# succinctlabs/sp1

Measured on NVIDIA H100. Metric: riscv_cycles_proven_per_second_core, higher is better.
Workload: dtype u32 KoalaBear (Montgomery) / ext4

## Files before the change

### sp1_b200/csrc/zerocheck.cu

```cuda
#include "ctx.cuh"
#include "challenger.cuh"
#include "hostfield.hpp"
#include "kb31.cuh"
#include <algorithm>
#include <memory>
#include <vector>

#include "machine.cuh"
#include "zc_lower.hpp"
#include "sumcheck.cuh"

namespace {

using kb::Ext;
using hf::E4;

constexpr int ZC_BLOCK = 128;
constexpr int ZC_LOCAL_REGS = 128;
constexpr int ZC_GLOBAL_REGS = 1024;
constexpr unsigned ZC_GLOBAL_MAXB = 132 * 2;
constexpr size_t ZC_MAX_PIECES = 16;

template <class K> struct Ops;
template <> struct Ops<uint32_t> {
    static __device__ __forceinline__ uint32_t zero() { return 0; }
    static __device__ __forceinline__ uint32_t from_base(uint32_t x) { return x; }
    static __device__ __forceinline__ uint32_t add(uint32_t a, uint32_t b) { return kb::add(a, b); }
    static __device__ __forceinline__ uint32_t sub(uint32_t a, uint32_t b) { return kb::sub(a, b); }
    static __device__ __forceinline__ uint32_t mul(uint32_t a, uint32_t b) { return kb::mul(a, b); }
    static __device__ __forceinline__ uint32_t load(const uint32_t* p, uint64_t i) { return __ldg(p + i); }
    static __device__ __forceinline__ Ext scale(const Ext& e, uint32_t k) { return kb::ext_mul_base(e, k); }
};
template <> struct Ops<Ext> {
    static __device__ __forceinline__ Ext zero() { return kb::ext_zero(); }
    static __device__ __forceinline__ Ext from_base(uint32_t x) { return kb::ext_from_base(x); }
    static __device__ __forceinline__ Ext add(const Ext& a, const Ext& b) { return kb::ext_add(a, b); }
    static __device__ __forceinline__ Ext sub(const Ext& a, const Ext& b) { return kb::ext_sub(a, b); }
    static __device__ __forceinline__ Ext mul(const Ext& a, const Ext& b) { return kb::ext_mul(a, b); }
    static __device__ __forceinline__ Ext load(const Ext* p, uint64_t i) { return kb::ext_load(reinterpret_cast<const uint32_t*>(p + i)); }
    static __device__ __forceinline__ Ext scale(const Ext& e, const Ext& k) { return kb::ext_mul(e, k); }
};

struct ZcJob {
    const void* main; const void* prep; const uint32_t* alpha_pows; uint64_t h;
    uint32_t blk_start, nblk, chip, columns;
    uint32_t zc_begin, zc_end;
    const void* batch;
};
static_assert(sizeof(ZcJob) == 64, "ZcJob layout");
struct ZcFixJob {
    const void* main; const void* prep; uint32_t* out; uint64_t h;
    uint32_t main_w, prep_w, blk_start, pad;
};

template <class J>
__device__ __forceinline__ int find_job(const J* __restrict__ jobs, int n, uint32_t blk) {
    int lo = 0, hi = n - 1;
    while (lo < hi) {
        int mid = (lo + hi + 1) >> 1;
        if (jobs[mid].blk_start <= blk) lo = mid; else hi = mid - 1;
    }
    return lo;
}

enum { RF_SMEM = 0, RF_LOCAL = 1, RF_GLOBAL = 2 };
template <class K, int RF, int NODES = 3> struct RegFile;
template <class K, int NODES> struct RegFile<K, RF_SMEM, NODES> {
    K* base;
    __device__ __forceinline__ RegFile(unsigned char* smem, void*, uint32_t) : base(reinterpret_cast<K*>(smem) + threadIdx.x) {}
    __device__ __forceinline__ K get(uint32_t r, int n) const { return base[(r * NODES + n) * ZC_BLOCK]; }
    __device__ __forceinline__ void set(uint32_t r, int n, const K& v) { base[(r * NODES + n) * ZC_BLOCK] = v; }
};
template <class K, int NODES> struct RegFile<K, RF_LOCAL, NODES> {
    K regs[ZC_LOCAL_REGS * NODES];
    __device__ __forceinline__ RegFile(unsigned char*, void*, uint32_t) {}
    __device__ __forceinline__ K get(uint32_t r, int n) const { return regs[r * NODES + n]; }
    __device__ __forceinline__ void set(uint32_t r, int n, const K& v) { regs[r * NODES + n] = v; }
};
template <class K, int NODES> struct RegFile<K, RF_GLOBAL, NODES> {
    K* base;
    __device__ __forceinline__ RegFile(unsigned char*, void* ws, uint32_t ws_regs)
        : base(static_cast<K*>(ws) + (size_t)blockIdx.x * ws_regs * NODES * ZC_BLOCK + threadIdx.x) {}
    __device__ __forceinline__ K get(uint32_t r, int n) const { return base[(size_t)(r * NODES + n) * ZC_BLOCK]; }
    __device__ __forceinline__ void set(uint32_t r, int n, const K& v) { base[(size_t)(r * NODES + n) * ZC_BLOCK] = v; }
};

template <class K, int N0>
__device__ __forceinline__ void load_nodes(const K* __restrict__ base, uint32_t col, uint64_t h, uint64_t i, K (&v)[3]) {
    using O = Ops<K>;
    const K* c = base + (uint64_t)col * h;
    const K z = O::load(c, 2 * i);
    const K o = (2 * i + 1 < h) ? O::load(c, 2 * i + 1) : O::zero();
    const K d = O::sub(o, z);
    const K d2 = O::add(d, d);
    if (N0 == 0) v[0] = z;
    v[1] = O::add(z, d2);
    v[2] = O::add(v[1], d2);
}

template <class K, int RF, bool FIRST>
__global__ void __launch_bounds__(ZC_BLOCK) zc_sum_kernel(const ZcJob* __restrict__ jobs, int n_jobs, const ChipProg* __restrict__ chips,
                                                          const uint32_t* __restrict__ pv, const uint32_t* __restrict__ gkr_pows,
                                                          const uint32_t* __restrict__ E, uint32_t* __restrict__ partial,
                                                          void* __restrict__ ws, uint32_t ws_regs) {
    using O = Ops<K>;
    constexpr int N0 = FIRST ? 1 : 0;
    extern __shared__ __align__(16) unsigned char zc_smem[];
    __shared__ uint32_t red[5][4][ZC_BLOCK / 32];
    const ZcJob job = jobs[find_job(jobs, n_jobs, blockIdx.x)];
    const ChipProg& prog = chips[job.chip];
    const K* main = static_cast<const K*>(job.main);
    const K* prep = static_cast<const K*>(job.prep);
    const uint64_t h = job.h;
    const uint64_t terms = (h + 1) / 2;
    RegFile<K, RF> rf(zc_smem, ws, ws_regs);
    Ext acc[5];
#pragma unroll
    for (int a = 0; a < 5; a++) acc[a] = kb::ext_zero();
    const ZcInstr* __restrict__ zc = prog.zc + job.zc_begin;
    const uint32_t n_zc = job.zc_end - job.zc_begin;
    for (uint64_t i = (uint64_t)(blockIdx.x - job.blk_start) * ZC_BLOCK + threadIdx.x; i < terms; i += (uint64_t)job.nblk * ZC_BLOCK) {
        const Ext e = kb::ext_load(E + 4 * i);
        Ext row[3] = {kb::ext_zero(), kb::ext_zero(), kb::ext_zero()};
        ZcInstr in = n_zc ? zc[0] : ZcInstr{};
        for (uint32_t pc = 0; pc < n_zc; pc++) {
            const ZcInstr nxt = zc[pc + 1 < n_zc ? pc + 1 : pc];
            switch (in.op) {
                case ZC_LOAD_MAIN: case ZC_LOAD_PREP: {
                    K v[3];
                    load_nodes<K, N0>(in.op == ZC_LOAD_MAIN ? main : prep, (uint32_t)in.a | ((uint32_t)in.b << 16), h, i, v);
#pragma unroll
                    for (int n = N0; n < 3; n++) rf.set(in.out, n, v[n]);
                    break;
                }
                case ZC_CONST: { const K c = O::from_base(prog.consts[in.a]);
#pragma unroll
                    for (int n = N0; n < 3; n++) rf.set(in.out, n, c);
                    break; }
                case ZC_PUBLIC: { const K c = O::from_base(pv[prog.publics[in.a]]);
#pragma unroll
                    for (int n = N0; n < 3; n++) rf.set(in.out, n, c);
                    break; }
                case ZC_ADD: {
                    K r[3];
#pragma unroll
                    for (int n = N0; n < 3; n++) r[n] = O::add(rf.get(in.a, n), rf.get(in.b, n));
#pragma unroll
                    for (int n = N0; n < 3; n++) rf.set(in.out, n, r[n]);
                    break; }
                case ZC_SUB: {
                    K r[3];
#pragma unroll
                    for (int n = N0; n < 3; n++) r[n] = O::sub(rf.get(in.a, n), rf.get(in.b, n));
#pragma unroll
                    for (int n = N0; n < 3; n++) rf.set(in.out, n, r[n]);
                    break; }
                case ZC_MUL: {
                    K r[3];
#pragma unroll
                    for (int n = N0; n < 3; n++) r[n] = O::mul(rf.get(in.a, n), rf.get(in.b, n));
#pragma unroll
                    for (int n = N0; n < 3; n++) rf.set(in.out, n, r[n]);
                    break; }
                case ZC_NEG: {
                    K r[3];
#pragma unroll
                    for (int n = N0; n < 3; n++) r[n] = O::sub(O::zero(), rf.get(in.a, n));
#pragma unroll
                    for (int n = N0; n < 3; n++) rf.set(in.out, n, r[n]);
                    break; }
                case ZC_ASSERT: {
                    const Ext al = kb::ext_load(job.alpha_pows + 4 * in.b);
#pragma unroll
                    for (int n = N0; n < 3; n++) row[n] = kb::ext_add(row[n], O::scale(al, rf.get(in.a, n)));
                    break; }
                default: __trap();
            }
            in = nxt;
        }
#pragma unroll
        for (int n = N0; n < 3; n++) acc[n] = kb::ext_add(acc[n], kb::ext_mul(row[n], e));
        if (!job.columns) continue;
        Ext s0 = kb::ext_zero(), s1 = kb::ext_zero();
        const bool has_o = 2 * i + 1 < h;
        if (job.batch) {
            const uint32_t* B = static_cast<const uint32_t*>(job.batch);
            acc[3] = kb::ext_add(acc[3], kb::ext_mul(kb::ext_load(B + 8 * i), e));
            if (has_o) acc[4] = kb::ext_add(acc[4], kb::ext_mul(kb::ext_load(B + 8 * i + 4), e));
            continue;
        }
        for (uint32_t j = 0; j < prog.main_w; j++) {
            const Ext g = kb::ext_load(gkr_pows + 4 * j);
            const K* c = main + (uint64_t)j * h;
            s0 = kb::ext_add(s0, O::scale(g, O::load(c, 2 * i)));
            if (has_o) s1 = kb::ext_add(s1, O::scale(g, O::load(c, 2 * i + 1)));
        }
        for (uint32_t j = 0; j < prog.prep_w; j++) {
            const Ext g = kb::ext_load(gkr_pows + 4 * (prog.main_w + j));
            const K* c = prep + (uint64_t)j * h;
            s0 = kb::ext_add(s0, O::scale(g, O::load(c, 2 * i)));
            if (has_o) s1 = kb::ext_add(s1, O::scale(g, O::load(c, 2 * i + 1)));
        }
        acc[3] = kb::ext_add(acc[3], kb::ext_mul(s0, e));
        acc[4] = kb::ext_add(acc[4], kb::ext_mul(s1, e));
    }
    const int lane = threadIdx.x & 31, warp = threadIdx.x >> 5;
#pragma unroll
    for (int a = 0; a < 5; a++)
#pragma unroll
        for (int l = 0; l < 4; l++) {
            uint32_t v = acc[a].c[l];
            for (int s = 16; s > 0; s >>= 1) v = kb::add(v, __shfl_down_sync(0xffffffffu, v, s));
            if (lane == 0) red[a][l][warp] = v;
        }
    __syncthreads();
    if (threadIdx.x < 36) {
        const int node = threadIdx.x / 12, slot = (threadIdx.x >> 2) % 3, l = threadIdx.x & 3;
        const int a = slot == 0 ? node : (node == 0 ? 2 + slot : -1);
        uint32_t v = 0;
        if (a >= 0)
            for (int w = 0; w < ZC_BLOCK / 32; w++) v = kb::add(v, red[a][l][w]);
        partial[(uint64_t)blockIdx.x * 36 + threadIdx.x] = v;
    }
}

__global__ void __launch_bounds__(128) zc_reduce_kernel(const ZcJob* __restrict__ jobs, const uint32_t* __restrict__ partial, uint32_t* __restrict__ out,
                                                        Mail mail) {
    const ZcJob job = jobs[blockIdx.x];
    __shared__ uint32_t red[36][4];
    const int slot = threadIdx.x >> 2, part = threadIdx.x & 3;
    for (int w = slot; w < 36; w += 32) {
        uint32_t v = 0;
        for (uint32_t b = part; b < job.nblk; b += 4) v = kb::add(v, partial[(uint64_t)(job.blk_start + b) * 36 + w]);
        red[w][part] = v;
    }
    __syncthreads();
    if (threadIdx.x < 36) {
        const uint32_t* r = red[threadIdx.x];
        out[blockIdx.x * 36 + threadIdx.x] = kb::add(kb::add(r[0], r[1]), kb::add(r[2], r[3]));
    }
    sp1_mail_done(mail);
}

template <class K>
__global__ void __launch_bounds__(256) zc_fix_kernel(const ZcFixJob* __restrict__ jobs, int n_jobs, Ext alpha) {
    using O = Ops<K>;
    const ZcFixJob job = jobs[find_job(jobs, n_jobs, blockIdx.x)];
    const uint64_t h = job.h, nh = (h + 1) / 2;
    const uint32_t bpc = (uint32_t)((nh + 255) / 256);
    const uint32_t lb = blockIdx.x - job.blk_start;
    const uint64_t j = lb / bpc;
    const uint64_t i = (uint64_t)(lb - (uint32_t)j * bpc) * 256 + threadIdx.x;
    if (i >= nh) return;
    const uint64_t t = j * nh + i;
    const K* in = j < job.main_w ? static_cast<const K*>(job.main) + j * h : static_cast<const K*>(job.prep) + (j - job.main_w) * h;
    K a = O::load(in, 2 * i);
    K b = (2 * i + 1 < h) ? O::load(in, 2 * i + 1) : O::zero();
    Ext r;
    if constexpr (sizeof(K) == 4) r = kb::ext_add(kb::ext_from_base(a), kb::ext_mul_base(alpha, kb::sub(b, a)));
    else r = kb::ext_add(a, kb::ext_mul(alpha, kb::ext_sub(b, a)));
    kb::ext_store(job.out + 4 * t, r);
}

__global__ void __launch_bounds__(256) zc_batch0_kernel(const ZcFixJob* __restrict__ jobs, int n_jobs, const uint32_t* __restrict__ gkr_pows, Ext alpha) {
    const ZcFixJob job = jobs[find_job(jobs, n_jobs, blockIdx.x)];
    const uint64_t h = job.h, nh = (h + 1) / 2;
    const uint64_t i = (uint64_t)(blockIdx.x - job.blk_start) * 256 + threadIdx.x;
    if (i >= nh) return;
    const bool has_o = 2 * i + 1 < h;
    Ext sa = kb::ext_zero(), sd = kb::ext_zero();
    const uint32_t* main = static_cast<const uint32_t*>(job.main);
    const uint32_t* prep = static_cast<const uint32_t*>(job.prep);
    for (uint32_t j = 0; j < job.main_w + job.prep_w; j++) {
        const uint32_t* c = j < job.main_w ? main + (uint64_t)j * h : prep + (uint64_t)(j - job.main_w) * h;
        const uint32_t a = __ldg(c + 2 * i), b = has_o ? __ldg(c + 2 * i + 1) : 0u;
        const Ext g = kb::ext_load(gkr_pows + 4 * j);
        sa = kb::ext_add(sa, kb::ext_mul_base(g, a));
        sd = kb::ext_add(sd, kb::ext_mul_base(g, kb::sub(b, a)));
    }
    kb::ext_store(job.out + 4 * i, kb::ext_add(sa, kb::ext_mul(alpha, sd)));
}

struct ZcDbgJob {
    const uint32_t* main; const uint32_t* prep; uint64_t h;
    const uint32_t* rows;
    uint32_t* out;
    uint32_t* count;
    uint32_t n, blk_start, nblk, chip, cwords, pad;
};
static_assert(sizeof(ZcDbgJob) == 72, "ZcDbgJob layout");

template <int RF, bool LISTED>
__global__ void __launch_bounds__(ZC_BLOCK) zc_debug_kernel(const ZcDbgJob* __restrict__ jobs, int n_jobs, const ChipProg* __restrict__ chips,
                                                            const uint32_t* __restrict__ pv, void* __restrict__ ws, uint32_t ws_regs) {
    extern __shared__ __align__(16) unsigned char zc_smem[];
    const ZcDbgJob job = jobs[find_job(jobs, n_jobs, blockIdx.x)];
    const ChipProg& prog = chips[job.chip];
    RegFile<uint32_t, RF, 1> rf(zc_smem, ws, ws_regs);
    const ZcInstr* __restrict__ zc = prog.zc;
    const uint32_t n_zc = prog.n_zc, lane = threadIdx.x & 31;
    for (uint64_t t0 = (uint64_t)(blockIdx.x - job.blk_start) * ZC_BLOCK + (threadIdx.x - lane); t0 < job.n; t0 += (uint64_t)job.nblk * ZC_BLOCK) {
        const uint64_t t = t0 + lane;
        bool fail = false;
        if (t < job.n) {
            const uint64_t row = LISTED ? job.rows[t] : t;
            for (uint32_t pc = 0; pc < n_zc; pc++) {
                const ZcInstr in = zc[pc];
                switch (in.op) {
                    case ZC_LOAD_MAIN: rf.set(in.out, 0, __ldg(job.main + (uint64_t)((uint32_t)in.a | ((uint32_t)in.b << 16)) * job.h + row)); break;
                    case ZC_LOAD_PREP: rf.set(in.out, 0, __ldg(job.prep + (uint64_t)((uint32_t)in.a | ((uint32_t)in.b << 16)) * job.h + row)); break;
                    case ZC_CONST: rf.set(in.out, 0, prog.consts[in.a]); break;
                    case ZC_PUBLIC: rf.set(in.out, 0, pv[prog.publics[in.a]]); break;
                    case ZC_ADD: rf.set(in.out, 0, kb::add(rf.get(in.a, 0), rf.get(in.b, 0))); break;
                    case ZC_SUB: rf.set(in.out, 0, kb::sub(rf.get(in.a, 0), rf.get(in.b, 0))); break;
                    case ZC_MUL: rf.set(in.out, 0, kb::mul(rf.get(in.a, 0), rf.get(in.b, 0))); break;
                    case ZC_NEG: rf.set(in.out, 0, kb::neg(rf.get(in.a, 0))); break;
                    case ZC_ASSERT:
                        if (rf.get(in.a, 0)) {
                            fail = true;
                            if (LISTED) job.out[t * job.cwords + (in.b >> 5)] |= 1u << (in.b & 31);
                        }
                        break;
                    default: __trap();
                }
            }
        }
        if (!LISTED) {
            const uint32_t bits = __ballot_sync(0xffffffffu, fail);
            if (lane == 0 && bits) { job.out[t0 >> 5] = bits; atomicAdd(job.count, (uint32_t)__popc(bits)); }
        }
    }
}

struct ZcDbgSelect { const uint32_t* bits; uint32_t* rows; uint32_t n_words, take; };
__global__ void __launch_bounds__(32) zc_debug_select_kernel(const ZcDbgSelect* __restrict__ jobs) {
    const ZcDbgSelect s = jobs[blockIdx.x];
    const uint32_t lane = threadIdx.x;
    uint32_t taken = 0;
    for (uint32_t w0 = 0; w0 < s.n_words && taken < s.take; w0 += 32) {
        uint32_t word = w0 + lane < s.n_words ? s.bits[w0 + lane] : 0u;
        const uint32_t c = __popc(word);
        uint32_t incl = c;
        for (int d = 1; d < 32; d <<= 1) {
            const uint32_t x = __shfl_up_sync(0xffffffffu, incl, d);
            if (lane >= (uint32_t)d) incl += x;
        }
        for (uint32_t rank = taken + incl - c; word && rank < s.take; rank++, word &= word - 1)
            s.rows[rank] = (w0 + lane) * 32 + (uint32_t)(__ffs(word) - 1);
        taken += __shfl_sync(0xffffffffu, incl, 31);
    }
}

E4 host_eval_zero_row(const HostProg& p, const uint32_t* pv, const std::vector<E4>& powers, uint32_t n_regs) {
    std::vector<uint32_t> regs(n_regs ? n_regs : 1, 0);
    for (const DagInstr& in : p.instrs) {
        switch (in.opcode) {
            case BC_LOAD_LEAF: regs[in.out] = 0; break;
            case BC_LOAD_CONST: regs[in.out] = p.consts[in.a]; break;
            case BC_LOAD_PUBLIC: regs[in.out] = pv[p.publics[in.a]]; break;
            case BC_ADD_F: regs[in.out] = hf::add(regs[in.a], regs[in.b]); break;
            case BC_SUB_F: regs[in.out] = hf::sub(regs[in.a], regs[in.b]); break;
            case BC_MUL_F: regs[in.out] = hf::mul(regs[in.a], regs[in.b]); break;
            case BC_NEG_F: regs[in.out] = hf::neg(regs[in.a]); break;
        }
    }
    E4 acc;
    for (size_t i = 0; i < p.assert_regs.size(); i++) acc = acc + powers[p.assert_alphas[i]] * regs[p.assert_regs[i]];
    return acc;
}

struct VGeq {
    uint32_t threshold = 0; E4 geq_c, eq_c;
    VGeq fix_last(const E4& a) const {
        VGeq r; r.threshold = threshold >> 1; r.geq_c = geq_c;
        r.eq_c = (threshold & 1) == 0 ? (E4::one() - a) * eq_c : a * (eq_c + geq_c) - geq_c;
        return r;
    }
    E4 at(uint64_t idx) const { return idx < threshold ? E4() : (idx == threshold ? eq_c + geq_c : geq_c); }
};

}

sp1b200_machine::~sp1b200_machine() {
    if (interactions) sp1b200_free_interactions(interactions);
    cudaFree(d_arena);
    cudaFree(d_zc_arena);
    cudaFree(d_chips);
}

extern "C" {

sp1b200_err sp1b200_machine_create(sp1b200_ctx* ctx, const uint32_t* h_blob, uint64_t n_words, sp1b200_machine** out) { SP1_DEVICE_GUARD(ctx);
    auto m = std::make_unique<sp1b200_machine>();
    SP1_CUDA(cudaMalloc((void**)&m->d_arena, n_words * 4 + 16));
    SP1_CUDA(cudaMemcpyAsync(m->d_arena, h_blob, n_words * 4, cudaMemcpyHostToDevice, ctx->stream));
    const uint32_t* b = h_blob;
    const uint32_t* end = h_blob + n_words;
    auto dev = [&](const uint32_t* hp) { return m->d_arena + (hp - h_blob); };
    if (n_words < 1 || !h_blob) return sp1b200_set_error("machine_create: empty blob");
    uint32_t n = *b++;
    for (uint32_t c = 0; c < n; c++) {
        if ((uint64_t)(end - b) < 9) return sp1b200_set_error("machine_create: truncated blob (header of chip %u)", c);
        ChipProg p{}; HostProg hp;
        p.main_w = *b++; p.prep_w = *b++; p.n_constraints = *b++; p.n_regs = *b++;
        const uint64_t ni = *b++, nl = *b++, nc = *b++, np = *b++, na = *b++;
        if (2 * ni + 2 * nl + nc + np + 2 * na > (uint64_t)(end - b)) return sp1b200_set_error("machine_create: truncated blob (chip %u)", c);
        if (p.n_regs > 65536) return sp1b200_set_error("machine_create: chip %u declares %u registers (16-bit register indices)", c, p.n_regs);
        p.n_instrs = (uint32_t)ni; p.n_asserts = (uint32_t)na;
        p.instrs = reinterpret_cast<const DagInstr*>(dev(b)); hp.instrs.resize(ni); memcpy(hp.instrs.data(), b, ni * 8); b += 2 * ni;
        p.leaves = reinterpret_cast<const LeafRef*>(dev(b)); hp.leaves.resize(nl); memcpy(hp.leaves.data(), b, nl * 8); b += 2 * nl;
        p.consts = dev(b); hp.consts.assign(b, b + nc); b += nc;
        p.publics = dev(b); hp.publics.assign(b, b + np); b += np;
        p.assert_regs = dev(b); hp.assert_regs.assign(b, b + na); b += na;
        p.assert_alphas = dev(b); hp.assert_alphas.assign(b, b + na); b += na;
        for (const LeafRef& l : hp.leaves) {
            if (l.source != LEAF_MAIN && l.source != LEAF_PREP) return sp1b200_set_error("machine_create: chip %u: leaf source %u (expected 2 = preprocessed or 4 = main)", c, l.source);
            if (l.col >= (l.source == LEAF_MAIN ? p.main_w : p.prep_w)) return sp1b200_set_error("machine_create: chip %u: leaf column %u outside the %s width", c, l.col, l.source == LEAF_MAIN ? "main" : "preprocessed");
        }
        for (size_t k = 0; k < hp.instrs.size(); k++) {
            const DagInstr& in = hp.instrs[k];
            if (in.out >= p.n_regs) return sp1b200_set_error("machine_create: chip %u instr %zu: output register %u >= n_regs %u", c, k, in.out, p.n_regs);
            bool ok = true;
            switch (in.opcode) {
                case BC_LOAD_LEAF: ok = in.a < nl; break;
                case BC_LOAD_CONST: ok = in.a < nc; break;
                case BC_LOAD_PUBLIC: ok = in.a < np; break;
                case BC_ADD_F: case BC_SUB_F: case BC_MUL_F: ok = in.a < p.n_regs && in.b < p.n_regs; break;
                case BC_NEG_F: ok = in.a < p.n_regs; break;
                default: return sp1b200_set_error("machine_create: chip %u instr %zu: unknown opcode %u", c, k, in.opcode);
            }
            if (!ok) return sp1b200_set_error("machine_create: chip %u instr %zu: operand out of range (opcode %u, a %u, b %u)", c, k, in.opcode, in.a, in.b);
        }
        for (size_t k = 0; k < hp.assert_regs.size(); k++) {
            if (hp.assert_regs[k] >= p.n_regs) return sp1b200_set_error("machine_create: chip %u assert %zu: register %u >= n_regs %u", c, k, hp.assert_regs[k], p.n_regs);
            if (hp.assert_alphas[k] >= p.n_constraints) return sp1b200_set_error("machine_create: chip %u assert %zu: alpha index %u >= n_constraints %u", c, k, hp.assert_alphas[k], p.n_constraints);
        }
        m->chips.push_back(p); m->host.push_back(std::move(hp));
    }
    {
        std::vector<uint32_t> widths;
        for (auto& c : m->chips) { widths.push_back(c.main_w); widths.push_back(c.prep_w); }
        widths.push_back(0);
        m->interactions = sp1b200_parse_interactions(b, end, n, widths.data());
        if (!m->interactions) return sp1b200_last_error();
    }
    std::vector<ZcInstr> all;
    std::vector<size_t> zc_off(n);
    for (uint32_t c = 0; c < n; c++) {
        ZcLowered L = zc_lower(m->host[c]);
        if (!L.error.empty()) return sp1b200_set_error("machine_create: chip %u: %s", c, L.error.c_str());
        zc_off[c] = all.size();
        m->chips[c].n_zc = (uint32_t)L.instrs.size();
        m->chips[c].zc_regs = L.n_regs;
        all.insert(all.end(), L.instrs.begin(), L.instrs.end());
        const size_t na = m->host[c].assert_regs.size();
        const size_t np_ = std::min<size_t>(ZC_MAX_PIECES, na / 4);
        if (np_ >= 2 && L.instrs.size() >= 128) {
            for (size_t q = 0; q < np_; q++) {
                ZcLowered P = zc_lower(m->host[c], 24, na * q / np_, na * (q + 1) / np_);
                if (!P.error.empty()) return sp1b200_set_error("machine_create: chip %u: %s", c, P.error.c_str());
                m->host[c].zc_pieces.emplace_back((uint32_t)(all.size() - zc_off[c]), (uint32_t)P.instrs.size());
                m->chips[c].zc_regs = std::max(m->chips[c].zc_regs, P.n_regs);
                all.insert(all.end(), P.instrs.begin(), P.instrs.end());
            }
        }
    }
    SP1_CUDA(cudaMalloc(&m->d_zc_arena, all.size() * sizeof(ZcInstr) + 16));
    if (!all.empty()) SP1_CUDA(cudaMemcpyAsync(m->d_zc_arena, all.data(), all.size() * sizeof(ZcInstr), cudaMemcpyHostToDevice, ctx->stream));
    for (uint32_t c = 0; c < n; c++) m->chips[c].zc = static_cast<const ZcInstr*>(m->d_zc_arena) + zc_off[c];
    SP1_CUDA(cudaMalloc((void**)&m->d_chips, (n ? n : 1) * sizeof(ChipProg)));
    if (n) SP1_CUDA(cudaMemcpyAsync(m->d_chips, m->chips.data(), n * sizeof(ChipProg), cudaMemcpyHostToDevice, ctx->stream));
    SP1_CUDA(cudaStreamSynchronize(ctx->stream));
    *out = m.release();
    return nullptr;
}
void sp1b200_machine_free(sp1b200_ctx*, sp1b200_machine* m) { delete m; }
uint32_t sp1b200_machine_chip_regs(const sp1b200_machine* m, uint32_t chip) { return chip < m->chips.size() ? m->chips[chip].zc_regs : 0; }
uint32_t sp1b200_machine_num_chips(const sp1b200_machine* m) { return (uint32_t)m->chips.size(); }

sp1b200_err sp1b200_zerocheck(sp1b200_ctx* ctx, const sp1b200_machine* m, const uint64_t* h_heights, const uint32_t* const* d_main,
                              const uint32_t* const* d_prep, const uint32_t* h_pv, uint32_t n_pv, const uint32_t* h_gkr_point,
                              const uint32_t* h_alpha, const uint32_t* h_gamma, const uint32_t* h_claims, uint32_t* h_chal, uint32_t* h_out,
                              uint64_t cap, uint64_t* h_words) { SP1_DEVICE_GUARD(ctx);
    const uint32_t mlr = ctx->params.max_log_row_count;
    const size_t nchips = m->chips.size();
    for (size_t k = 0; k < nchips; k++)
        for (uint32_t pi : m->host[k].publics)
            if (pi >= n_pv) return sp1b200_set_error("zerocheck: chip %zu reads public value %u but only %u were passed", k, pi, n_pv);
    cudaStream_t st = ctx->stream;
    DevFree mem(ctx);
    HostChallenger ch;
    SP1_TRY(ch.init(ctx, h_chal));
    PhaseTimer t_all(ctx, "zerocheck.total");
    HostAccum acc_wait(ctx, "zerocheck.host_wait"), acc_math(ctx, "zerocheck.host_math"), acc_setup(ctx, "zerocheck.host_setup");
    auto t_setup = std::make_unique<HostSpan>(acc_setup);
    const E4 alpha = E4::load(h_alpha), gamma = E4::load(h_gamma);

    struct St {
        uint64_t h;
        std::vector<E4> zeta; E4 eq_adj = E4::one(), pra; VGeq vg;
    };
    std::vector<St> S(nchips);
    size_t maxc = 0, maxw = 0, total_w = 0, total_c = 0;
    for (auto& c : m->chips) {
        maxc = std::max<size_t>(maxc, c.n_constraints); maxw = std::max<size_t>(maxw, c.main_w + c.prep_w);
        total_w += c.main_w + c.prep_w; total_c += c.n_constraints ? c.n_constraints : 1;
    }
    std::vector<E4> pw(maxc ? maxc : 1); pw[0] = E4::one();
    for (size_t i = 1; i < pw.size(); i++) pw[i] = pw[i - 1] * alpha;
    std::vector<E4> gw(maxw ? maxw : 1); gw[0] = gamma;
    for (size_t i = 1; i < gw.size(); i++) gw[i] = gw[i - 1] * gamma;
    uint32_t *d_pv, *d_gw, *d_ap;
    SP1_TRY(mem.alloc((void**)&d_pv, (n_pv ? n_pv : 1) * 4));
    if (n_pv) SP1_CUDA(cudaMemcpyAsync(d_pv, h_pv, n_pv * 4, cudaMemcpyHostToDevice, st));
    SP1_TRY(mem.alloc((void**)&d_gw, gw.size() * 16));
    SP1_CUDA(cudaMemcpyAsync(d_gw, gw.data(), gw.size() * 16, cudaMemcpyHostToDevice, st));
    std::vector<E4> gp(mlr);
    for (uint32_t i = 0; i < mlr; i++) gp[i] = E4::load(h_gkr_point + 4 * i);
    std::vector<E4> all_ap; all_ap.reserve(total_c);
    std::vector<size_t> ap_off(nchips), woff(nchips);
    std::vector<uint64_t> boff0(nchips), boff1(nchips);
    uint64_t b0 = 0, b1 = 0; size_t wsum = 0;
    for (size_t k = 0; k < nchips; k++) {
        const ChipProg& p = m->chips[k];
        St& s = S[k];
        s.h = h_heights[k];
        if (s.h > ((uint64_t)1 << mlr)) return sp1b200_set_error("zerocheck: chip %zu height exceeds 2^%u", k, mlr);
        if (p.zc_regs > ZC_GLOBAL_REGS) return sp1b200_set_error("zerocheck: chip %zu needs %u live registers (> %d)", k, p.zc_regs, ZC_GLOBAL_REGS);
        s.zeta = gp;
        std::vector<E4> rev(pw.begin(), pw.begin() + p.n_constraints);
        std::reverse(rev.begin(), rev.end());
        ap_off[k] = all_ap.size();
        all_ap.insert(all_ap.end(), rev.begin(), rev.end());
        if (rev.empty()) all_ap.push_back(E4());
        s.pra = host_eval_zero_row(m->host[k], h_pv, rev, p.n_regs);
        s.vg.threshold = (uint32_t)s.h; s.vg.geq_c = E4::one();
        const uint64_t nh = (s.h + 1) / 2;
        const size_t w = p.main_w + p.prep_w;
        boff0[k] = b0; b0 += (uint64_t)(w + 1) * nh * 4;
        boff1[k] = b1; b1 += (uint64_t)(w + 1) * ((nh + 1) / 2) * 4;
        woff[k] = wsum; wsum += w;
    }
    SP1_TRY(mem.alloc((void**)&d_ap, all_ap.size() * 16));
    SP1_CUDA(cudaMemcpyAsync(d_ap, all_ap.data(), all_ap.size() * 16, cudaMemcpyHostToDevice, st));
    uint32_t *d_buf[2], *d_final;
    SP1_TRY(mem.alloc((void**)&d_buf[0], b0 * 4 + 16));
    SP1_TRY(mem.alloc((void**)&d_buf[1], b1 * 4 + 16));
    SP1_TRY(mem.alloc((void**)&d_final, (wsum ? wsum : 1) * 16));
    uint32_t *d_point, *d_E[2];
    SP1_TRY(mem.alloc((void**)&d_point, mlr * 16));
    SP1_CUDA(cudaMemcpyAsync(d_point, h_gkr_point, mlr * 16, cudaMemcpyHostToDevice, st));
    SP1_TRY(mem.alloc((void**)&d_E[0], ((size_t)16 << (mlr - 1))));
    SP1_TRY(mem.alloc((void**)&d_E[1], ((size_t)16 << (mlr > 1 ? mlr - 2 : 0))));
    SP1_TRY(launch_eq_table(ctx, d_point, (int)mlr - 1, d_E[0]));
    int ecur = 0;

    static const uint32_t TIER_REGS[3] = {8, 16, 32};
    auto tier_of = [&](uint32_t regs) { for (int t = 0; t < 3; t++) if (regs <= TIER_REGS[t]) return t; return regs <= (uint32_t)ZC_LOCAL_REGS ? 3 : 4; };
    size_t ws_bytes = 0;
    struct Launch { size_t job0; uint32_t n_jobs, blocks, regs; int tier; };
    struct RoundPlan { std::vector<Launch> sums; size_t fix0; uint32_t fix_jobs, fix_blocks; std::vector<uint32_t> chip_of_job; size_t job0; };
    std::vector<RoundPlan> plan(mlr);
    std::vector<ZcJob> jobs;
    std::vector<ZcFixJob> fjobs, bjobs;
    uint32_t batch_blocks = 0;
    const unsigned MAXB = 132 * 4;
    uint32_t max_blocks = 1, max_jobs = 1;
    {
        std::vector<uint64_t> hcur(nchips);
        for (size_t k = 0; k < nchips; k++) hcur[k] = S[k].h;
        for (uint32_t rd = 0; rd < mlr; rd++) {
            RoundPlan& R = plan[rd];
            R.job0 = jobs.size();
            auto in_main = [&](size_t k) -> const void* {
                if (rd == 0) return d_main[k];
                return (rd & 1 ? d_buf[0] + boff0[k] : d_buf[1] + boff1[k]);
            };
            auto in_prep = [&](size_t k) -> const void* {
                const ChipProg& p = m->chips[k];
                if (rd == 0) return p.prep_w ? d_prep[k] : nullptr;
                return static_cast<const uint32_t*>(in_main(k)) + (uint64_t)p.main_w * hcur[k] * 4;
            };
            auto in_batch = [&](size_t k) -> const void* {
                if (rd == 0) return nullptr;
                const ChipProg& p = m->chips[k];
                return static_cast<const uint32_t*>(in_main(k)) + (uint64_t)(p.main_w + p.prep_w) * hcur[k] * 4;
            };
            uint32_t blocks_round = 0;
            for (int tier = 0; tier < 5; tier++) {
                Launch Lc{jobs.size(), 0, 0, 0, tier};
                for (size_t k = 0; k < nchips; k++) {
                    const ChipProg& p = m->chips[k];
                    if (!hcur[k] || tier_of(p.zc_regs) != tier) continue;
                    unsigned nb = blocks_for((hcur[k] + 1) / 2, ZC_BLOCK);
                    if (nb > MAXB) nb = MAXB;
                    if (tier == 4 && nb > ZC_GLOBAL_MAXB) nb = ZC_GLOBAL_MAXB;
                    const auto& pieces = m->host[k].zc_pieces;
                    if (nb <= 16 && !pieces.empty()) {
                        for (size_t q = 0; q < pieces.size(); q++) {
                            ZcJob j{in_main(k), in_prep(k), d_ap + 4 * ap_off[k], hcur[k], Lc.blocks, nb, (uint32_t)k, q == 0 ? 1u : 0u,
                                    pieces[q].first, pieces[q].first + pieces[q].second, in_batch(k)};
                            jobs.push_back(j);
                            R.chip_of_job.push_back((uint32_t)k);
                            Lc.n_jobs++; Lc.blocks += nb;
                        }
                    } else {
                        ZcJob j{in_main(k), in_prep(k), d_ap + 4 * ap_off[k], hcur[k], Lc.blocks, nb, (uint32_t)k, 1u, 0u, p.n_zc, in_batch(k)};
                        jobs.push_back(j);
                        R.chip_of_job.push_back((uint32_t)k);
                        Lc.n_jobs++; Lc.blocks += nb;
                    }
                    Lc.regs = std::max(Lc.regs, p.zc_regs);
                }
                if (Lc.n_jobs) {
                    R.sums.push_back(Lc); blocks_round += Lc.blocks;
                    if (tier == 4) ws_bytes = std::max(ws_bytes, (size_t)Lc.blocks * Lc.regs * 3 * ZC_BLOCK * 16);
                }
            }
            max_blocks = std::max(max_blocks, blocks_round);
            max_jobs = std::max<uint32_t>(max_jobs, (uint32_t)R.chip_of_job.size());
            R.fix0 = fjobs.size(); R.fix_jobs = 0; R.fix_blocks = 0;
            for (size_t k = 0; k < nchips; k++) {
                const ChipProg& p = m->chips[k];
                if (!hcur[k]) continue;
                const uint64_t nh = (hcur[k] + 1) / 2;
                uint32_t* out = rd + 1 == mlr ? d_final + 4 * woff[k] : (rd & 1 ? d_buf[1] + boff1[k] : d_buf[0] + boff0[k]);
                const uint32_t fold_b = (rd > 0 && rd + 1 < mlr) ? 1u : 0u;
                ZcFixJob f{in_main(k), in_prep(k), out, hcur[k], p.main_w, p.prep_w + fold_b, R.fix_blocks, 0};
                fjobs.push_back(f);
                R.fix_jobs++; R.fix_blocks += blocks_for(nh, 256) * (p.main_w + p.prep_w + fold_b);
                if (rd == 0 && mlr > 1) {
                    ZcFixJob bj{d_main[k], m->chips[k].prep_w ? d_prep[k] : nullptr, d_buf[0] + boff0[k] + (uint64_t)(p.main_w + p.prep_w) * nh * 4, hcur[k],
                                p.main_w, p.prep_w, batch_blocks, 0};
                    bjobs.push_back(bj);
                    batch_blocks += blocks_for(nh, 256);
                }
                hcur[k] = nh;
            }
        }
    }
    ZcJob* d_jobs; ZcFixJob *d_fjobs, *d_bjobs; uint32_t *d_partial, *d_sums;
    SP1_TRY(mem.alloc((void**)&d_jobs, (jobs.size() + 1) * sizeof(ZcJob)));
    SP1_TRY(mem.alloc((void**)&d_fjobs, (fjobs.size() + 1) * sizeof(ZcFixJob)));
    SP1_TRY(mem.alloc((void**)&d_bjobs, (bjobs.size() + 1) * sizeof(ZcFixJob)));
    if (!bjobs.empty()) SP1_CUDA(cudaMemcpyAsync(d_bjobs, bjobs.data(), bjobs.size() * sizeof(ZcFixJob), cudaMemcpyHostToDevice, st));
    if (!jobs.empty()) SP1_CUDA(cudaMemcpyAsync(d_jobs, jobs.data(), jobs.size() * sizeof(ZcJob), cudaMemcpyHostToDevice, st));
    if (!fjobs.empty()) SP1_CUDA(cudaMemcpyAsync(d_fjobs, fjobs.data(), fjobs.size() * sizeof(ZcFixJob), cudaMemcpyHostToDevice, st));
    SP1_TRY(mem.alloc((void**)&d_partial, (size_t)max_blocks * 36 * 4));
    if ((size_t)max_jobs * 36 > SP1_MAIL_WORDS) return sp1b200_set_error("zerocheck: %u chips exceed the mailbox payload", max_jobs);
    d_sums = sp1b200_mail_dev(ctx);
    SP1_CUDA(cudaMemsetAsync(d_final, 0, (wsum ? wsum : 1) * 16, st));
    void* d_ws = nullptr;
    if (ws_bytes) SP1_TRY(mem.alloc(&d_ws, ws_bytes));
    auto launch_sum = [&](const Launch& Lc, bool ext, uint32_t* part) -> sp1b200_err {
        auto go = [&](auto kern, size_t smem) -> sp1b200_err {
            if (smem > 32 * 1024) SP1_CUDA(cudaFuncSetAttribute(kern, cudaFuncAttributeMaxDynamicSharedMemorySize, (int)smem));
            SP1_LAUNCH(ctx, kern, Lc.blocks, ZC_BLOCK, smem, d_jobs + Lc.job0, (int)Lc.n_jobs, m->d_chips, d_pv, d_gw, d_E[ecur], part, d_ws,
                       Lc.regs);
            return nullptr;
        };
        if (Lc.tier == 4) return ext ? go(zc_sum_kernel<Ext, RF_GLOBAL, false>, 0) : go(zc_sum_kernel<uint32_t, RF_GLOBAL, true>, 0);
        if (Lc.tier == 3) return ext ? go(zc_sum_kernel<Ext, RF_LOCAL, false>, 0) : go(zc_sum_kernel<uint32_t, RF_LOCAL, true>, 0);
        const size_t regs = Lc.regs;
        return ext ? go(zc_sum_kernel<Ext, RF_SMEM, false>, regs * 3 * ZC_BLOCK * 16) : go(zc_sum_kernel<uint32_t, RF_SMEM, true>, regs * 3 * ZC_BLOCK * 4);
    };

    t_setup.reset();
    E4 lambda; ch.sample_ext(lambda.c);
    std::vector<E4> round_claims(nchips);
    E4 claimed_sum;
    for (size_t k = 0; k < nchips; k++) { round_claims[k] = E4::load(h_claims + 4 * k); claimed_sum = claimed_sum * lambda + round_claims[k]; }
    std::vector<uint32_t> words;
    words.push_back(mlr);
    std::vector<E4> point;
    std::vector<E4> ys((size_t)nchips * 4);
    std::vector<uint32_t> hs((size_t)max_jobs * 36);
    std::vector<E4> chip_sums(nchips * 9);
    const E4 two = E4::from_base(hf::to_monty(2)), four = E4::from_base(hf::to_monty(4)), three = E4::from_base(hf::to_monty(3));
    for (uint32_t rd = 0; rd < mlr; rd++) {
        const RoundPlan& R = plan[rd];
        {
            uint32_t blk = 0, seq = 0; size_t jb = 0;
            for (const Launch& Lc : R.sums) {
                SP1_TRY(launch_sum(Lc, rd > 0, d_partial + (size_t)blk * 36));
                const Mail mail = sp1b200_mail_next(ctx); seq = mail.seq;
                SP1_LAUNCH(ctx, zc_reduce_kernel, Lc.n_jobs, 128, 0, d_jobs + Lc.job0, d_partial + (size_t)blk * 36, d_sums + jb * 36, mail);
                blk += Lc.blocks; jb += Lc.n_jobs;
            }
            if (jb) {
                HostSpan sp(acc_wait);
                SP1_TRY(sp1b200_mail_wait(ctx, seq));
                memcpy(hs.data(), sp1b200_mail_host(ctx), jb * 36 * 4);
            }
        }
        HostSpan sp_math(acc_math);
        std::fill(chip_sums.begin(), chip_sums.end(), E4());
        for (size_t j = 0; j < R.chip_of_job.size(); j++)
            for (int w9 = 0; w9 < 9; w9++) chip_sums[(size_t)R.chip_of_job[j] * 9 + w9] = chip_sums[(size_t)R.chip_of_job[j] * 9 + w9] + E4::load(&hs[j * 36 + 4 * w9]);
        const E4 last = gp[mlr - 1 - rd];
        const E4 bnode = (E4::one() - last) * hf::inv(E4::one() - (last + last));
        const E4 nodes[5] = {E4(), E4::one(), two, four, bnode};
        E4 basis[5][5];
        hf::lagrange_basis<5>(nodes, basis);
        const E4 f0 = E4::one() - last, f2 = last * hf::to_monty(3) - E4::one(), f4 = last * hf::to_monty(7) - three;
        E4 Y[4];
        for (size_t k = 0; k < nchips; k++) {
            St& s = S[k];
            E4* y = &ys[4 * k];
            if (s.h == 0) { y[0] = y[1] = y[2] = y[3] = E4(); }
            else {
                const E4* q = &chip_sums[k * 9];
                const E4 A = q[1], B = q[2];
                E4 y0 = q[0] + A;
                E4 y2 = q[3] + (B + B) - A;
                E4 y4 = q[6] + B * four - A * three;
                const uint64_t th = (s.h + 1) / 2 - 1;
                const uint64_t esize = (uint64_t)1 << (s.zeta.size() - 1);
                E4 eth;
                if (th < esize) {
                    const size_t kk = s.zeta.size() - 1;
                    eth = E4::one();
                    for (size_t t = 0; t < kk; t++) eth = eth * (((th >> (kk - 1 - t)) & 1) ? s.zeta[t] : E4::one() - s.zeta[t]);
                }
                const E4 msb = s.eq_adj * eth;
                const E4 v0 = s.vg.fix_last(E4()).at(th), v2 = s.vg.fix_last(two).at(th), v4 = s.vg.fix_last(four).at(th);
                y0 = y0 * (f0 * s.eq_adj) - s.pra * v0 * msb * f0;
                y2 = y2 * (f2 * s.eq_adj) - s.pra * v2 * msb * f2;
                y4 = y4 * (f4 * s.eq_adj) - s.pra * v4 * msb * f4;
                y[0] = y0; y[1] = round_claims[k] - y0; y[2] = y2; y[3] = y4;
            }
            for (int i = 0; i < 4; i++) Y[i] = (k ? Y[i] * lambda : E4()) + y[i];
        }
        E4 rlc[5];
        for (int c5 = 0; c5 < 5; c5++) for (int i = 0; i < 4; i++) rlc[c5] = rlc[c5] + basis[i][c5] * Y[i];
        for (auto& c : rlc) ch.observe_n(c.c, 4);
        words.push_back(5);
        for (auto& c : rlc) words.insert(words.end(), c.c, c.c + 4);
        E4 a; ch.sample_ext(a.c);
        point.insert(point.begin(), a);
        const Ext da = to_ext(a);
        if (R.fix_jobs) {
            if (rd == 0) {
                SP1_LAUNCH(ctx, zc_fix_kernel<uint32_t>, R.fix_blocks, 256, 0, d_fjobs + R.fix0, (int)R.fix_jobs, da);
                if (!bjobs.empty()) SP1_LAUNCH(ctx, zc_batch0_kernel, batch_blocks, 256, 0, d_bjobs, (int)bjobs.size(), d_gw, da);
            } else SP1_LAUNCH(ctx, zc_fix_kernel<Ext>, R.fix_blocks, 256, 0, d_fjobs + R.fix0, (int)R.fix_jobs, da);
        }
        E4 La[4];
        for (int i = 0; i < 4; i++) La[i] = hf::eval_poly<5>(basis[i], a);
        for (size_t k = 0; k < nchips; k++) {
            St& s = S[k];
            const E4* y = &ys[4 * k];
            round_claims[k] = y[0] * La[0] + y[1] * La[1] + y[2] * La[2] + y[3] * La[3];
            s.vg = s.vg.fix_last(a);
            if (s.h == 0) continue;
            s.eq_adj = s.eq_adj * (a * last + (E4::one() - a) * (E4::one() - last));
            s.zeta.pop_back();
            s.h = (s.h + 1) / 2;
        }
        if (rd + 1 < mlr) {
            const uint64_t n_out = (uint64_t)1 << (mlr - 2 - rd);
            SP1_TRY(launch_halve_eq(ctx, d_E[ecur], n_out, d_E[ecur ^ 1]));
            ecur ^= 1;
        }
    }
    E4 final_eval;
    for (auto& c : round_claims) final_eval = final_eval * lambda + c;
    words.insert(words.end(), claimed_sum.c, claimed_sum.c + 4);
    for (auto& x : point) words.insert(words.end(), x.c, x.c + 4);
    words.insert(words.end(), final_eval.c, final_eval.c + 4);
    std::vector<uint32_t> fin((wsum ? wsum : 1) * 4);
    SP1_CUDA(cudaMemcpyAsync(fin.data(), d_final, fin.size() * 4, cudaMemcpyDeviceToHost, st));
    SP1_CUDA(cudaStreamSynchronize(st));
    ch.observe(hf::to_monty(nchips));
    for (size_t k = 0; k < nchips; k++) {
        const ChipProg& p = m->chips[k];
        const uint32_t* mv = &fin[4 * woff[k]];
        const uint32_t* pvv = mv + 4 * (size_t)p.main_w;
        ch.observe(hf::to_monty(p.prep_w)); ch.observe_n(pvv, (size_t)p.prep_w * 4);
        ch.observe(hf::to_monty(p.main_w)); ch.observe_n(mv, (size_t)p.main_w * 4);
        words.insert(words.end(), pvv, pvv + (size_t)p.prep_w * 4);
        words.insert(words.end(), mv, mv + (size_t)p.main_w * 4);
    }
    t_all.stop();
    ch.store(h_chal);
    if (h_words) *h_words = words.size();
    if (words.size() > cap) return sp1b200_set_error("zerocheck: output needs %zu words, capacity %llu", words.size(), (unsigned long long)cap);
    if (h_out) memcpy(h_out, words.data(), words.size() * 4);
    return nullptr;
}

}

sp1b200_err sp1b200_debug_constraints_device(sp1b200_ctx* ctx, const sp1b200_machine* m, const uint64_t* h_heights, const uint32_t* const* d_main,
                                             const uint32_t* const* d_prep, const uint32_t* h_pv, uint32_t n_pv, uint32_t max_rows,
                                             std::vector<uint32_t>& words) {
    const size_t nchips = m->chips.size();
    for (size_t k = 0; k < nchips; k++) {
        for (uint32_t pi : m->host[k].publics)
            if (pi >= n_pv) return sp1b200_set_error("debug_constraints: chip %zu reads public value %u but only %u were passed", k, pi, n_pv);
        if (m->chips[k].zc_regs > ZC_GLOBAL_REGS)
            return sp1b200_set_error("debug_constraints: chip %zu needs %u live registers (> %d)", k, m->chips[k].zc_regs, ZC_GLOBAL_REGS);
    }
    cudaStream_t st = ctx->stream;
    DevFree mem(ctx);
    PhaseTimer t_all(ctx, "debug_constraints.total");
    uint32_t* d_pv;
    SP1_TRY(mem.alloc((void**)&d_pv, (n_pv ? n_pv : 1) * 4));
    if (n_pv) SP1_CUDA(cudaMemcpyAsync(d_pv, h_pv, n_pv * 4, cudaMemcpyHostToDevice, st));
    static const uint32_t TIER_REGS[3] = {8, 16, 32};
    auto tier_of = [&](uint32_t regs) { for (int t = 0; t < 3; t++) if (regs <= TIER_REGS[t]) return t; return regs <= (uint32_t)ZC_LOCAL_REGS ? 3 : 4; };
    struct Launch { size_t job0; uint32_t n_jobs, blocks, regs; int tier; };
    auto plan = [&](std::vector<ZcDbgJob>& jobs, std::vector<Launch>& launches, size_t& ws_bytes, auto n_of, auto fill) {
        for (int tier = 0; tier < 5; tier++) {
            Launch Lc{jobs.size(), 0, 0, 0, tier};
            for (size_t k = 0; k < nchips; k++) {
                const uint64_t n = n_of(k);
                if (!n || tier_of(m->chips[k].zc_regs) != tier) continue;
                unsigned nb = std::min<unsigned>(blocks_for(n, ZC_BLOCK), 132 * 4);
                if (tier == 4) nb = std::min(nb, ZC_GLOBAL_MAXB);
                ZcDbgJob j{};
                j.main = d_main[k]; j.prep = m->chips[k].prep_w ? d_prep[k] : nullptr; j.h = h_heights[k];
                j.n = (uint32_t)n; j.blk_start = Lc.blocks; j.nblk = nb; j.chip = (uint32_t)k;
                fill(k, j);
                jobs.push_back(j);
                Lc.n_jobs++; Lc.blocks += nb; Lc.regs = std::max(Lc.regs, m->chips[k].zc_regs);
            }
            if (Lc.n_jobs) {
                launches.push_back(Lc);
                if (tier == 4) ws_bytes = std::max(ws_bytes, (size_t)Lc.blocks * Lc.regs * ZC_BLOCK * 4);
            }
        }
    };
    auto run = [&](const std::vector<ZcDbgJob>& jobs, const std::vector<Launch>& launches, size_t ws_bytes, bool listed) -> sp1b200_err {
        ZcDbgJob* d_jobs;
        void* d_ws = nullptr;
        SP1_TRY(mem.alloc((void**)&d_jobs, (jobs.size() + 1) * sizeof(ZcDbgJob)));
        if (!jobs.empty()) SP1_CUDA(cudaMemcpyAsync(d_jobs, jobs.data(), jobs.size() * sizeof(ZcDbgJob), cudaMemcpyHostToDevice, st));
        if (ws_bytes) SP1_TRY(mem.alloc(&d_ws, ws_bytes));
        for (const Launch& Lc : launches) {
            auto go = [&](auto kern, size_t smem) -> sp1b200_err {
                SP1_LAUNCH(ctx, kern, Lc.blocks, ZC_BLOCK, smem, d_jobs + Lc.job0, (int)Lc.n_jobs, m->d_chips, d_pv, d_ws, Lc.regs);
                return nullptr;
            };
            sp1b200_err e;
            if (Lc.tier == 4) e = listed ? go(zc_debug_kernel<RF_GLOBAL, true>, 0) : go(zc_debug_kernel<RF_GLOBAL, false>, 0);
            else if (Lc.tier == 3) e = listed ? go(zc_debug_kernel<RF_LOCAL, true>, 0) : go(zc_debug_kernel<RF_LOCAL, false>, 0);
            else e = listed ? go(zc_debug_kernel<RF_SMEM, true>, (size_t)Lc.regs * ZC_BLOCK * 4)
                            : go(zc_debug_kernel<RF_SMEM, false>, (size_t)Lc.regs * ZC_BLOCK * 4);
            SP1_TRY(e);
        }
        return nullptr;
    };

    std::vector<uint64_t> bm_off(nchips);
    uint64_t bm_words = 0;
    for (size_t k = 0; k < nchips; k++) { bm_off[k] = bm_words; bm_words += (h_heights[k] + 31) / 32; }
    uint32_t *d_bm, *d_cnt;
    SP1_TRY(mem.alloc((void**)&d_bm, (bm_words ? bm_words : 1) * 4));
    SP1_TRY(mem.alloc((void**)&d_cnt, (nchips ? nchips : 1) * 4));
    SP1_CUDA(cudaMemsetAsync(d_bm, 0, (bm_words ? bm_words : 1) * 4, st));
    SP1_CUDA(cudaMemsetAsync(d_cnt, 0, (nchips ? nchips : 1) * 4, st));
    {
        std::vector<ZcDbgJob> jobs; std::vector<Launch> launches; size_t ws = 0;
        plan(jobs, launches, ws, [&](size_t k) { return h_heights[k]; },
             [&](size_t k, ZcDbgJob& j) { j.out = d_bm + bm_off[k]; j.count = d_cnt + k; });
        SP1_TRY(run(jobs, launches, ws, false));
    }
    std::vector<uint32_t> cnt(nchips);
    if (nchips) SP1_CUDA(cudaMemcpyAsync(cnt.data(), d_cnt, nchips * 4, cudaMemcpyDeviceToHost, st));
    SP1_CUDA(cudaStreamSynchronize(st));

    std::vector<uint64_t> row_off(nchips), cbm_off(nchips);
    std::vector<uint32_t> take(nchips), cwords(nchips);
    uint64_t n_rows = 0, n_cbm = 0;
    std::vector<ZcDbgSelect> sel;
    uint32_t* d_rows;
    for (size_t k = 0; k < nchips; k++) {
        take[k] = std::min(cnt[k], max_rows);
        cwords[k] = (m->chips[k].n_constraints + 31) / 32;
        row_off[k] = n_rows; n_rows += take[k];
        cbm_off[k] = n_cbm; n_cbm += (uint64_t)take[k] * cwords[k];
    }
    SP1_TRY(mem.alloc((void**)&d_rows, (n_rows ? n_rows : 1) * 4));
    std::vector<uint32_t> rows(n_rows), cbm(n_cbm);
    if (n_rows) {
        for (size_t k = 0; k < nchips; k++)
            if (take[k]) sel.push_back(ZcDbgSelect{d_bm + bm_off[k], d_rows + row_off[k], (uint32_t)((h_heights[k] + 31) / 32), take[k]});
        ZcDbgSelect* d_sel;
        uint32_t* d_cbm;
        SP1_TRY(mem.alloc((void**)&d_sel, sel.size() * sizeof(ZcDbgSelect)));
        SP1_TRY(mem.alloc((void**)&d_cbm, (n_cbm ? n_cbm : 1) * 4));
        SP1_CUDA(cudaMemcpyAsync(d_sel, sel.data(), sel.size() * sizeof(ZcDbgSelect), cudaMemcpyHostToDevice, st));
        SP1_CUDA(cudaMemsetAsync(d_cbm, 0, (n_cbm ? n_cbm : 1) * 4, st));
        SP1_LAUNCH(ctx, zc_debug_select_kernel, (unsigned)sel.size(), 32, 0, d_sel);
        std::vector<ZcDbgJob> jobs; std::vector<Launch> launches; size_t ws = 0;
        plan(jobs, launches, ws, [&](size_t k) { return (uint64_t)take[k]; },
             [&](size_t k, ZcDbgJob& j) { j.rows = d_rows + row_off[k]; j.out = d_cbm + cbm_off[k]; j.cwords = cwords[k]; });
        SP1_TRY(run(jobs, launches, ws, true));
        SP1_CUDA(cudaMemcpyAsync(rows.data(), d_rows, n_rows * 4, cudaMemcpyDeviceToHost, st));
        if (n_cbm) SP1_CUDA(cudaMemcpyAsync(cbm.data(), d_cbm, n_cbm * 4, cudaMemcpyDeviceToHost, st));
        SP1_CUDA(cudaStreamSynchronize(st));
    }
    t_all.stop();
    words.assign(1, 0);
    for (size_t k = 0; k < nchips; k++) {
        if (!cnt[k]) continue;
        words[0]++;
        words.push_back((uint32_t)k); words.push_back(cnt[k]); words.push_back(take[k]);
        for (uint32_t i = 0; i < take[k]; i++) {
            words.push_back(rows[row_off[k] + i]);
            const size_t n_at = words.size();
            words.push_back(0);
            const uint32_t* b = &cbm[cbm_off[k] + (uint64_t)i * cwords[k]];
            for (uint32_t c = 0; c < m->chips[k].n_constraints; c++)
                if ((b[c >> 5] >> (c & 31)) & 1) { words.push_back(c); words[n_at]++; }
        }
    }
    return nullptr;
}
```

Measured before the change: 64.76 million.

## Evaluate first two zerocheck rounds on a 2D grid in one base-field pass

Adds a grid kernel that reads four rows at once and evaluates constraints on a 2D node grid, so round 0 and round 1 sums both come from a single base-field pass over the trace. The host derives both rounds' univariate evaluations from 16 accumulated sums. A fold2 kernel then folds two variables at once, replacing the separate round-0 fix, the batch0 kernel, the round-1 extension-field sum pass and one eq-halving. The cost is six nodes per interpreter pass, done twice, which means more register or shared-memory pressure and more interpreted work in the first round.

```diff
diff --git a/sp1_b200/csrc/zc_grid.hpp b/sp1_b200/csrc/zc_grid.hpp
--- /dev/null
+++ b/sp1_b200/csrc/zc_grid.hpp
@@ -0,0 +1,29 @@
+#pragma once
+#include "hostfield.hpp"
+#include <cstdint>
+
+inline void zc_grid_round0(const hf::E4* g, const hf::E4& z, uint64_t h, const hf::E4& pad, hf::E4* out) {
+    using hf::E4;
+    const E4 z0 = E4::one() - z;
+    const E4 skip = (h % 4 == 1 || h % 4 == 2) ? z * pad : E4();
+    for (int i = 0; i < 9; i++) out[i] = E4();
+    out[3] = z0 * g[0] + z * g[1] - skip;
+    out[6] = z0 * g[4] + z * g[5] - skip;
+    out[1] = z0 * g[12] + z * g[14];
+    out[2] = z0 * g[13] + z * g[15];
+}
+
+inline void zc_grid_round1(const hf::E4* g, const hf::E4& a0, uint64_t h, const hf::E4& pad, hf::E4* out) {
+    using hf::E4;
+    const E4 nodes[4] = {E4(), E4::one(), E4::from_base(hf::to_monty(2)), E4::from_base(hf::to_monty(4))};
+    E4 basis[4][4];
+    hf::lagrange_basis<4>(nodes, basis);
+    E4 L[4];
+    for (int i = 0; i < 4; i++) L[i] = hf::eval_poly<4>(basis[i], a0);
+    for (int i = 0; i < 9; i++) out[i] = E4();
+    out[0] = L[2] * g[0] + L[3] * g[4] + (h % 4 == 1 ? L[1] * pad : E4());
+    out[3] = L[0] * g[8] + L[1] * g[10] + L[2] * g[2] + L[3] * g[6];
+    out[6] = L[0] * g[9] + L[1] * g[11] + L[2] * g[3] + L[3] * g[7];
+    out[1] = g[12] + a0 * (g[13] - g[12]);
+    out[2] = g[14] + a0 * (g[15] - g[14]);
+}
diff --git a/sp1_b200/csrc/zerocheck.cu b/sp1_b200/csrc/zerocheck.cu
--- a/sp1_b200/csrc/zerocheck.cu
+++ b/sp1_b200/csrc/zerocheck.cu
@@ -8,6 +8,7 @@
 
 #include "machine.cuh"
 #include "zc_lower.hpp"
+#include "zc_grid.hpp"
 #include "sumcheck.cuh"
 
 namespace {
@@ -51,6 +52,7 @@
 struct ZcFixJob {
     const void* main; const void* prep; uint32_t* out; uint64_t h;
     uint32_t main_w, prep_w, blk_start, pad;
+    const uint32_t* corners;
 };
 
 template <class J>
@@ -98,6 +100,70 @@
     v[2] = O::add(v[1], d2);
 }
 
+template <class K, int RF, int NODES, int N0, class Load>
+__device__ __forceinline__ void zc_interpret(const ZcJob& job, const ChipProg& prog, const uint32_t* __restrict__ pv,
+                                             RegFile<K, RF, NODES>& rf, const Load& load, Ext (&row)[NODES]) {
+    using O = Ops<K>;
+    const ZcInstr* __restrict__ zc = prog.zc + job.zc_begin;
+    const uint32_t n_zc = job.zc_end - job.zc_begin;
+    ZcInstr in = n_zc ? zc[0] : ZcInstr{};
+    for (uint32_t pc = 0; pc < n_zc; pc++) {
+        const ZcInstr nxt = zc[pc + 1 < n_zc ? pc + 1 : pc];
+        switch (in.op) {
+            case ZC_LOAD_MAIN: case ZC_LOAD_PREP: {
+                K v[NODES];
+                load(in.op == ZC_LOAD_MAIN, (uint32_t)in.a | ((uint32_t)in.b << 16), v);
+#pragma unroll
+                for (int n = N0; n < NODES; n++) rf.set(in.out, n, v[n]);
+                break;
+            }
+            case ZC_CONST: { const K c = O::from_base(prog.consts[in.a]);
+#pragma unroll
+                for (int n = N0; n < NODES; n++) rf.set(in.out, n, c);
+                break; }
+            case ZC_PUBLIC: { const K c = O::from_base(pv[prog.publics[in.a]]);
+#pragma unroll
+                for (int n = N0; n < NODES; n++) rf.set(in.out, n, c);
+                break; }
+            case ZC_ADD: {
+                K r[NODES];
+#pragma unroll
+                for (int n = N0; n < NODES; n++) r[n] = O::add(rf.get(in.a, n), rf.get(in.b, n));
+#pragma unroll
+                for (int n = N0; n < NODES; n++) rf.set(in.out, n, r[n]);
+                break; }
+            case ZC_SUB: {
+                K r[NODES];
+#pragma unroll
+                for (int n = N0; n < NODES; n++) r[n] = O::sub(rf.get(in.a, n), rf.get(in.b, n));
+#pragma unroll
+                for (int n = N0; n < NODES; n++) rf.set(in.out, n, r[n]);
+                break; }
+            case ZC_MUL: {
+                K r[NODES];
+#pragma unroll
+                for (int n = N0; n < NODES; n++) r[n] = O::mul(rf.get(in.a, n), rf.get(in.b, n));
+#pragma unroll
+                for (int n = N0; n < NODES; n++) rf.set(in.out, n, r[n]);
+                break; }
+            case ZC_NEG: {
+                K r[NODES];
+#pragma unroll
+                for (int n = N0; n < NODES; n++) r[n] = O::sub(O::zero(), rf.get(in.a, n));
+#pragma unroll
+                for (int n = N0; n < NODES; n++) rf.set(in.out, n, r[n]);
+                break; }
+            case ZC_ASSERT: {
+                const Ext al = kb::ext_load(job.alpha_pows + 4 * in.b);
+#pragma unroll
+                for (int n = N0; n < NODES; n++) row[n] = kb::ext_add(row[n], O::scale(al, rf.get(in.a, n)));
+                break; }
+            default: __trap();
+        }
+        in = nxt;
+    }
+}
+
 template <class K, int RF, bool FIRST>
 __global__ void __launch_bounds__(ZC_BLOCK) zc_sum_kernel(const ZcJob* __restrict__ jobs, int n_jobs, const ChipProg* __restrict__ chips,
                                                           const uint32_t* __restrict__ pv, const uint32_t* __restrict__ gkr_pows,
@@ -117,67 +183,11 @@
     Ext acc[5];
 #pragma unroll
     for (int a = 0; a < 5; a++) acc[a] = kb::ext_zero();
-    const ZcInstr* __restrict__ zc = prog.zc + job.zc_begin;
-    const uint32_t n_zc = job.zc_end - job.zc_begin;
     for (uint64_t i = (uint64_t)(blockIdx.x - job.blk_start) * ZC_BLOCK + threadIdx.x; i < terms; i += (uint64_t)job.nblk * ZC_BLOCK) {
         const Ext e = kb::ext_load(E + 4 * i);
         Ext row[3] = {kb::ext_zero(), kb::ext_zero(), kb::ext_zero()};
-        ZcInstr in = n_zc ? zc[0] : ZcInstr{};
-        for (uint32_t pc = 0; pc < n_zc; pc++) {
-            const ZcInstr nxt = zc[pc + 1 < n_zc ? pc + 1 : pc];
-            switch (in.op) {
-                case ZC_LOAD_MAIN: case ZC_LOAD_PREP: {
-                    K v[3];
-                    load_nodes<K, N0>(in.op == ZC_LOAD_MAIN ? main : prep, (uint32_t)in.a | ((uint32_t)in.b << 16), h, i, v);
-#pragma unroll
-                    for (int n = N0; n < 3; n++) rf.set(in.out, n, v[n]);
-                    break;
-                }
-                case ZC_CONST: { const K c = O::from_base(prog.consts[in.a]);
-#pragma unroll
-                    for (int n = N0; n < 3; n++) rf.set(in.out, n, c);
-                    break; }
-                case ZC_PUBLIC: { const K c = O::from_base(pv[prog.publics[in.a]]);
-#pragma unroll
-                    for (int n = N0; n < 3; n++) rf.set(in.out, n, c);
-                    break; }
-                case ZC_ADD: {
-                    K r[3];
-#pragma unroll
-                    for (int n = N0; n < 3; n++) r[n] = O::add(rf.get(in.a, n), rf.get(in.b, n));
-#pragma unroll
-                    for (int n = N0; n < 3; n++) rf.set(in.out, n, r[n]);
-                    break; }
-                case ZC_SUB: {
-                    K r[3];
-#pragma unroll
-                    for (int n = N0; n < 3; n++) r[n] = O::sub(rf.get(in.a, n), rf.get(in.b, n));
-#pragma unroll
-                    for (int n = N0; n < 3; n++) rf.set(in.out, n, r[n]);
-                    break; }
-                case ZC_MUL: {
-                    K r[3];
-#pragma unroll
-                    for (int n = N0; n < 3; n++) r[n] = O::mul(rf.get(in.a, n), rf.get(in.b, n));
-#pragma unroll
-                    for (int n = N0; n < 3; n++) rf.set(in.out, n, r[n]);
-                    break; }
-                case ZC_NEG: {
-                    K r[3];
-#pragma unroll
-                    for (int n = N0; n < 3; n++) r[n] = O::sub(O::zero(), rf.get(in.a, n));
-#pragma unroll
-                    for (int n = N0; n < 3; n++) rf.set(in.out, n, r[n]);
-                    break; }
-                case ZC_ASSERT: {
-                    const Ext al = kb::ext_load(job.alpha_pows + 4 * in.b);
-#pragma unroll
-                    for (int n = N0; n < 3; n++) row[n] = kb::ext_add(row[n], O::scale(al, rf.get(in.a, n)));
-                    break; }
-                default: __trap();
-            }
-            in = nxt;
-        }
+        zc_interpret<K, RF, 3, N0>(job, prog, pv, rf, [&](bool is_main, uint32_t col, K (&v)[3]) { load_nodes<K, N0>(is_main ? main : prep, col, h, i, v); },
+                                   row);
 #pragma unroll
         for (int n = N0; n < 3; n++) acc[n] = kb::ext_add(acc[n], kb::ext_mul(row[n], e));
         if (!job.columns) continue;
@@ -224,20 +234,122 @@
     }
 }
 
+constexpr int ZC_GRID_WORDS = 64;
+constexpr int ZC_GRID_NODES = 6;
+template <int RF>
+__global__ void __launch_bounds__(ZC_BLOCK, 3) zc_grid_kernel(const ZcJob* __restrict__ jobs, int n_jobs, const ChipProg* __restrict__ chips,
+                                                           const uint32_t* __restrict__ pv, const uint32_t* __restrict__ gkr_pows,
+                                                           const uint32_t* __restrict__ E, uint32_t* __restrict__ partial,
+                                                           void* __restrict__ ws, uint32_t ws_regs) {
+    extern __shared__ __align__(16) unsigned char zc_smem[];
+    const ZcJob job = jobs[find_job(jobs, n_jobs, blockIdx.x)];
+    const ChipProg& prog = chips[job.chip];
+    const uint32_t* main = static_cast<const uint32_t*>(job.main);
+    const uint32_t* prep = static_cast<const uint32_t*>(job.prep);
+    const uint64_t h = job.h;
+    const uint64_t terms = (h + 3) / 4;
+    RegFile<uint32_t, RF, ZC_GRID_NODES> rf(zc_smem, ws, ws_regs);
+    Ext acc[16];
+#pragma unroll
+    for (int a = 0; a < 16; a++) acc[a] = kb::ext_zero();
+    for (uint64_t q = (uint64_t)(blockIdx.x - job.blk_start) * ZC_BLOCK + threadIdx.x; q < terms; q += (uint64_t)job.nblk * ZC_BLOCK) {
+        const Ext e = kb::ext_load(E + 4 * q);
+        const uint64_t r0 = 4 * q;
+        auto quad = [&](const uint32_t* c, uint32_t (&v)[4]) {
+#pragma unroll
+            for (int t = 0; t < 4; t++) v[t] = r0 + t < h ? __ldg(c + r0 + t) : 0u;
+        };
+#pragma unroll
+        for (int pass = 0; pass < 2; pass++) {
+            Ext row[ZC_GRID_NODES];
+#pragma unroll
+            for (int n = 0; n < ZC_GRID_NODES; n++) row[n] = kb::ext_zero();
+            zc_interpret<uint32_t, RF, ZC_GRID_NODES, 0>(job, prog, pv, rf, [&](bool is_main, uint32_t col, uint32_t (&v)[ZC_GRID_NODES]) {
+                uint32_t c[4];
+                quad((is_main ? main : prep) + (uint64_t)col * h, c);
+                const uint32_t d0 = kb::sub(c[1], c[0]), d1 = kb::sub(c[3], c[2]);
+                const uint32_t x0 = kb::add(d0, d0), x1 = kb::add(d1, d1);
+                const uint32_t a = kb::add(c[0], pass ? kb::add(x0, x0) : x0), b = kb::add(c[2], pass ? kb::add(x1, x1) : x1);
+                const uint32_t d = kb::sub(b, a), d2 = kb::add(d, d);
+                v[0] = a; v[1] = b; v[2] = kb::add(a, d2); v[3] = kb::add(v[2], d2);
+                const uint32_t dy = kb::sub(c[2 + pass], c[pass]), y2 = kb::add(dy, dy);
+                v[4] = kb::add(c[pass], y2); v[5] = kb::add(v[4], y2);
+            }, row);
+#pragma unroll
+            for (int n = 0; n < 4; n++) acc[4 * pass + n] = kb::ext_add(acc[4 * pass + n], kb::ext_mul(row[n], e));
+#pragma unroll
+            for (int n = 0; n < 2; n++) acc[8 + 2 * pass + n] = kb::ext_add(acc[8 + 2 * pass + n], kb::ext_mul(row[4 + n], e));
+        }
+        if (!job.columns) continue;
+        Ext s[4] = {kb::ext_zero(), kb::ext_zero(), kb::ext_zero(), kb::ext_zero()};
+        for (uint32_t j = 0; j < prog.main_w + prog.prep_w; j++) {
+            const Ext g = kb::ext_load(gkr_pows + 4 * j);
+            uint32_t c[4];
+            quad(j < prog.main_w ? main + (uint64_t)j * h : prep + (uint64_t)(j - prog.main_w) * h, c);
+#pragma unroll
+            for (int t = 0; t < 4; t++) s[t] = kb::ext_add(s[t], kb::ext_mul_base(g, c[t]));
+        }
+#pragma unroll
+        for (int t = 0; t < 4; t++) acc[12 + t] = kb::ext_add(acc[12 + t], kb::ext_mul(s[t], e));
+        if (job.batch) {
+            uint32_t* out = static_cast<uint32_t*>(const_cast<void*>(job.batch)) + 16 * q;
+#pragma unroll
+            for (int t = 0; t < 4; t++) kb::ext_store(out + 4 * t, s[t]);
+        }
+    }
+    block_reduce<16>(acc, partial, Mail{});
+}
+
+__global__ void __launch_bounds__(256) zc_fold2_kernel(const ZcFixJob* __restrict__ jobs, int n_jobs, Ext a0, Ext a1) {
+    const ZcFixJob job = jobs[find_job(jobs, n_jobs, blockIdx.x)];
+    const uint64_t h = job.h, nq = (h + 3) / 4;
+    const uint32_t bpc = (uint32_t)((nq + 255) / 256);
+    const uint32_t lb = blockIdx.x - job.blk_start;
+    const uint32_t j = lb / bpc;
+    const uint64_t q = (uint64_t)(lb - j * bpc) * 256 + threadIdx.x;
+    if (q >= nq) return;
+    const uint32_t w = job.main_w + job.prep_w;
+    const Ext a01 = kb::ext_mul(a0, a1);
+    auto col = [&](uint32_t k) {
+        return k < job.main_w ? static_cast<const uint32_t*>(job.main) + (uint64_t)k * h : static_cast<const uint32_t*>(job.prep) + (uint64_t)(k - job.main_w) * h;
+    };
+    auto coeffs = [&](uint32_t k, uint32_t (&d)[4]) {
+        const uint32_t* c = col(k);
+        uint32_t v[4];
+#pragma unroll
+        for (int t = 0; t < 4; t++) v[t] = 4 * q + t < h ? __ldg(c + 4 * q + t) : 0u;
+        d[0] = v[0]; d[1] = kb::sub(v[1], v[0]); d[2] = kb::sub(v[2], v[0]); d[3] = kb::sub(kb::sub(v[3], v[1]), d[2]);
+    };
+    Ext r;
+    if (j < w) {
+        uint32_t d[4];
+        coeffs(j, d);
+        r = kb::ext_add(kb::ext_add(kb::ext_from_base(d[0]), kb::ext_mul_base(a0, d[1])), kb::ext_add(kb::ext_mul_base(a1, d[2]), kb::ext_mul_base(a01, d[3])));
+    } else {
+        const uint32_t* c = job.corners + 16 * q;
+        const Ext s00 = kb::ext_load(c), s10 = kb::ext_load(c + 4), s01 = kb::ext_load(c + 8), s11 = kb::ext_load(c + 12);
+        const Ext d2 = kb::ext_sub(s01, s00);
+        const Ext d3 = kb::ext_sub(kb::ext_sub(s11, s10), d2);
+        r = kb::ext_add(kb::ext_add(s00, kb::ext_mul(a0, kb::ext_sub(s10, s00))), kb::ext_add(kb::ext_mul(a1, d2), kb::ext_mul(a01, d3)));
+    }
+    kb::ext_store(job.out + 4 * ((uint64_t)j * nq + q), r);
+}
+
+template <int WORDS>
 __global__ void __launch_bounds__(128) zc_reduce_kernel(const ZcJob* __restrict__ jobs, const uint32_t* __restrict__ partial, uint32_t* __restrict__ out,
                                                         Mail mail) {
     const ZcJob job = jobs[blockIdx.x];
-    __shared__ uint32_t red[36][4];
+    __shared__ uint32_t red[WORDS][4];
     const int slot = threadIdx.x >> 2, part = threadIdx.x & 3;
-    for (int w = slot; w < 36; w += 32) {
+    for (int w = slot; w < WORDS; w += 32) {
         uint32_t v = 0;
-        for (uint32_t b = part; b < job.nblk; b += 4) v = kb::add(v, partial[(uint64_t)(job.blk_start + b) * 36 + w]);
+        for (uint32_t b = part; b < job.nblk; b += 4) v = kb::add(v, partial[(uint64_t)(job.blk_start + b) * WORDS + w]);
         red[w][part] = v;
     }
     __syncthreads();
-    if (threadIdx.x < 36) {
+    if (threadIdx.x < WORDS) {
         const uint32_t* r = red[threadIdx.x];
-        out[blockIdx.x * 36 + threadIdx.x] = kb::add(kb::add(r[0], r[1]), kb::add(r[2], r[3]));
+        out[blockIdx.x * WORDS + threadIdx.x] = kb::add(kb::add(r[0], r[1]), kb::add(r[2], r[3]));
     }
     sp1_mail_done(mail);
 }
@@ -260,25 +372,6 @@
     if constexpr (sizeof(K) == 4) r = kb::ext_add(kb::ext_from_base(a), kb::ext_mul_base(alpha, kb::sub(b, a)));
     else r = kb::ext_add(a, kb::ext_mul(alpha, kb::ext_sub(b, a)));
     kb::ext_store(job.out + 4 * t, r);
-}
-
-__global__ void __launch_bounds__(256) zc_batch0_kernel(const ZcFixJob* __restrict__ jobs, int n_jobs, const uint32_t* __restrict__ gkr_pows, Ext alpha) {
-    const ZcFixJob job = jobs[find_job(jobs, n_jobs, blockIdx.x)];
-    const uint64_t h = job.h, nh = (h + 1) / 2;
-    const uint64_t i = (uint64_t)(blockIdx.x - job.blk_start) * 256 + threadIdx.x;
-    if (i >= nh) return;
-    const bool has_o = 2 * i + 1 < h;
-    Ext sa = kb::ext_zero(), sd = kb::ext_zero();
-    const uint32_t* main = static_cast<const uint32_t*>(job.main);
-    const uint32_t* prep = static_cast<const uint32_t*>(job.prep);
-    for (uint32_t j = 0; j < job.main_w + job.prep_w; j++) {
-        const uint32_t* c = j < job.main_w ? main + (uint64_t)j * h : prep + (uint64_t)(j - job.main_w) * h;
-        const uint32_t a = __ldg(c + 2 * i), b = has_o ? __ldg(c + 2 * i + 1) : 0u;
-        const Ext g = kb::ext_load(gkr_pows + 4 * j);
-        sa = kb::ext_add(sa, kb::ext_mul_base(g, a));
-        sd = kb::ext_add(sd, kb::ext_mul_base(g, kb::sub(b, a)));
-    }
-    kb::ext_store(job.out + 4 * i, kb::ext_add(sa, kb::ext_mul(alpha, sd)));
 }
 
 struct ZcDbgJob {
@@ -369,6 +462,13 @@
     return acc;
 }
 
+E4 eq_at(const std::vector<E4>& zeta, size_t kk, uint64_t idx) {
+    if (kk < 64 && idx >> kk) return E4();
+    E4 e = E4::one();
+    for (size_t t = 0; t < kk; t++) e = e * (((idx >> (kk - 1 - t)) & 1) ? zeta[t] : E4::one() - zeta[t]);
+    return e;
+}
+
 struct VGeq {
     uint32_t threshold = 0; E4 geq_c, eq_c;
     VGeq fix_last(const E4& a) const {
@@ -501,6 +601,7 @@
         std::vector<E4> zeta; E4 eq_adj = E4::one(), pra; VGeq vg;
     };
     std::vector<St> S(nchips);
+    const bool grid = mlr >= 2;
     size_t maxc = 0, maxw = 0, total_w = 0, total_c = 0;
     for (auto& c : m->chips) {
         maxc = std::max<size_t>(maxc, c.n_constraints); maxw = std::max<size_t>(maxw, c.main_w + c.prep_w);
@@ -519,8 +620,8 @@
     for (uint32_t i = 0; i < mlr; i++) gp[i] = E4::load(h_gkr_point + 4 * i);
     std::vector<E4> all_ap; all_ap.reserve(total_c);
     std::vector<size_t> ap_off(nchips), woff(nchips);
-    std::vector<uint64_t> boff0(nchips), boff1(nchips);
-    uint64_t b0 = 0, b1 = 0; size_t wsum = 0;
+    std::vector<uint64_t> boff0(nchips), boff1(nchips), coff(nchips);
+    uint64_t b0 = 0, b1 = 0, cw = 0; size_t wsum = 0;
     for (size_t k = 0; k < nchips; k++) {
         const ChipProg& p = m->chips[k];
         St& s = S[k];
@@ -535,10 +636,13 @@
         if (rev.empty()) all_ap.push_back(E4());
         s.pra = host_eval_zero_row(m->host[k], h_pv, rev, p.n_regs);
         s.vg.threshold = (uint32_t)s.h; s.vg.geq_c = E4::one();
-        const uint64_t nh = (s.h + 1) / 2;
+        const uint64_t nq = (s.h + 3) / 4;
         const size_t w = p.main_w + p.prep_w;
-        boff0[k] = b0; b0 += (uint64_t)(w + 1) * nh * 4;
-        boff1[k] = b1; b1 += (uint64_t)(w + 1) * ((nh + 1) / 2) * 4;
+        if (grid) {
+            boff0[k] = b0; b0 += (uint64_t)(w + 1) * ((nq + 1) / 2) * 4;
+            boff1[k] = b1; b1 += (uint64_t)(w + 1) * nq * 4;
+        }
+        coff[k] = cw; cw += nq * 16;
         woff[k] = wsum; wsum += w;
     }
     SP1_TRY(mem.alloc((void**)&d_ap, all_ap.size() * 16));
@@ -547,12 +651,16 @@
     SP1_TRY(mem.alloc((void**)&d_buf[0], b0 * 4 + 16));
     SP1_TRY(mem.alloc((void**)&d_buf[1], b1 * 4 + 16));
     SP1_TRY(mem.alloc((void**)&d_final, (wsum ? wsum : 1) * 16));
+    const bool keep_corners = grid && mlr > 2;
+    uint32_t* d_corners = nullptr;
+    if (keep_corners) SP1_TRY(mem.alloc((void**)&d_corners, cw * 4 + 16));
     uint32_t *d_point, *d_E[2];
+    const uint32_t e_bits = grid ? mlr - 2 : mlr - 1;
     SP1_TRY(mem.alloc((void**)&d_point, mlr * 16));
     SP1_CUDA(cudaMemcpyAsync(d_point, h_gkr_point, mlr * 16, cudaMemcpyHostToDevice, st));
-    SP1_TRY(mem.alloc((void**)&d_E[0], ((size_t)16 << (mlr - 1))));
-    SP1_TRY(mem.alloc((void**)&d_E[1], ((size_t)16 << (mlr > 1 ? mlr - 2 : 0))));
-    SP1_TRY(launch_eq_table(ctx, d_point, (int)mlr - 1, d_E[0]));
+    SP1_TRY(mem.alloc((void**)&d_E[0], ((size_t)16 << e_bits)));
+    SP1_TRY(mem.alloc((void**)&d_E[1], ((size_t)16 << (e_bits ? e_bits - 1 : 0))));
+    SP1_TRY(launch_eq_table(ctx, d_point, (int)e_bits, d_E[0]));
     int ecur = 0;
 
     static const uint32_t TIER_REGS[3] = {8, 16, 32};
@@ -562,8 +670,7 @@
     struct RoundPlan { std::vector<Launch> sums; size_t fix0; uint32_t fix_jobs, fix_blocks; std::vector<uint32_t> chip_of_job; size_t job0; };
     std::vector<RoundPlan> plan(mlr);
     std::vector<ZcJob> jobs;
-    std::vector<ZcFixJob> fjobs, bjobs;
-    uint32_t batch_blocks = 0;
+    std::vector<ZcFixJob> fjobs;
     const unsigned MAXB = 132 * 4;
     uint32_t max_blocks = 1, max_jobs = 1;
     {
@@ -582,21 +689,24 @@
                 return static_cast<const uint32_t*>(in_main(k)) + (uint64_t)p.main_w * hcur[k] * 4;
             };
             auto in_batch = [&](size_t k) -> const void* {
-                if (rd == 0) return nullptr;
+                if (rd == 0) return keep_corners ? d_corners + coff[k] : nullptr;
                 const ChipProg& p = m->chips[k];
                 return static_cast<const uint32_t*>(in_main(k)) + (uint64_t)(p.main_w + p.prep_w) * hcur[k] * 4;
             };
             uint32_t blocks_round = 0;
-            for (int tier = 0; tier < 5; tier++) {
+            const bool grid_pass = grid && rd == 0;
+            for (int tier = 0; tier < 5 && !(grid && rd == 1); tier++) {
                 Launch Lc{jobs.size(), 0, 0, 0, tier};
                 for (size_t k = 0; k < nchips; k++) {
                     const ChipProg& p = m->chips[k];
                     if (!hcur[k] || tier_of(p.zc_regs) != tier) continue;
-                    unsigned nb = blocks_for((hcur[k] + 1) / 2, ZC_BLOCK);
+                    unsigned nb = blocks_for(grid_pass ? (hcur[k] + 3) / 4 : (hcur[k] + 1) / 2, ZC_BLOCK);
                     if (nb > MAXB) nb = MAXB;
+                    if (grid_pass && nb > 132 * 3) nb = 132 * 3;
                     if (tier == 4 && nb > ZC_GLOBAL_MAXB) nb = ZC_GLOBAL_MAXB;
                     const auto& pieces = m->host[k].zc_pieces;
-                    if (nb <= 16 && !pieces.empty()) {
+                    const bool short_round = nb <= 16 || (!grid_pass && (hcur[k] + 1) / 2 <= 2ull * nb * ZC_BLOCK);
+                    if (short_round && !pieces.empty()) {
                         for (size_t q = 0; q < pieces.size(); q++) {
                             ZcJob j{in_main(k), in_prep(k), d_ap + 4 * ap_off[k], hcur[k], Lc.blocks, nb, (uint32_t)k, q == 0 ? 1u : 0u,
                                     pieces[q].first, pieces[q].first + pieces[q].second, in_batch(k)};
@@ -614,7 +724,7 @@
                 }
                 if (Lc.n_jobs) {
                     R.sums.push_back(Lc); blocks_round += Lc.blocks;
-                    if (tier == 4) ws_bytes = std::max(ws_bytes, (size_t)Lc.blocks * Lc.regs * 3 * ZC_BLOCK * 16);
+                    if (tier == 4) ws_bytes = std::max(ws_bytes, (size_t)Lc.blocks * Lc.regs * ZC_BLOCK * (grid_pass ? ZC_GRID_NODES * 4 : 3 * 16));
                 }
             }
             max_blocks = std::max(max_blocks, blocks_round);
@@ -625,40 +735,48 @@
                 if (!hcur[k]) continue;
                 const uint64_t nh = (hcur[k] + 1) / 2;
                 uint32_t* out = rd + 1 == mlr ? d_final + 4 * woff[k] : (rd & 1 ? d_buf[1] + boff1[k] : d_buf[0] + boff0[k]);
+                if (grid_pass) { hcur[k] = nh; continue; }
+                if (grid && rd == 1) {
+                    const uint32_t fold_b = rd + 1 < mlr ? 1u : 0u;
+                    ZcFixJob f{d_main[k], p.prep_w ? d_prep[k] : nullptr, out, S[k].h, p.main_w, p.prep_w, R.fix_blocks, fold_b,
+                               keep_corners ? d_corners + coff[k] : nullptr};
+                    fjobs.push_back(f);
+                    R.fix_jobs++; R.fix_blocks += blocks_for(nh, 256) * (p.main_w + p.prep_w + fold_b);
+                    hcur[k] = nh;
+                    continue;
+                }
                 const uint32_t fold_b = (rd > 0 && rd + 1 < mlr) ? 1u : 0u;
-                ZcFixJob f{in_main(k), in_prep(k), out, hcur[k], p.main_w, p.prep_w + fold_b, R.fix_blocks, 0};
+                ZcFixJob f{in_main(k), in_prep(k), out, hcur[k], p.main_w, p.prep_w + fold_b, R.fix_blocks, 0, nullptr};
                 fjobs.push_back(f);
                 R.fix_jobs++; R.fix_blocks += blocks_for(nh, 256) * (p.main_w + p.prep_w + fold_b);
-                if (rd == 0 && mlr > 1) {
-                    ZcFixJob bj{d_main[k], m->chips[k].prep_w ? d_prep[k] : nullptr, d_buf[0] + boff0[k] + (uint64_t)(p.main_w + p.prep_w) * nh * 4, hcur[k],
-                                p.main_w, p.prep_w, batch_blocks, 0};
-                    bjobs.push_back(bj);
-                    batch_blocks += blocks_for(nh, 256);
-                }
                 hcur[k] = nh;
             }
         }
     }
-    ZcJob* d_jobs; ZcFixJob *d_fjobs, *d_bjobs; uint32_t *d_partial, *d_sums;
+    ZcJob* d_jobs; ZcFixJob* d_fjobs; uint32_t *d_partial, *d_sums;
     SP1_TRY(mem.alloc((void**)&d_jobs, (jobs.size() + 1) * sizeof(ZcJob)));
     SP1_TRY(mem.alloc((void**)&d_fjobs, (fjobs.size() + 1) * sizeof(ZcFixJob)));
-    SP1_TRY(mem.alloc((void**)&d_bjobs, (bjobs.size() + 1) * sizeof(ZcFixJob)));
-    if (!bjobs.empty()) SP1_CUDA(cudaMemcpyAsync(d_bjobs, bjobs.data(), bjobs.size() * sizeof(ZcFixJob), cudaMemcpyHostToDevice, st));
     if (!jobs.empty()) SP1_CUDA(cudaMemcpyAsync(d_jobs, jobs.data(), jobs.size() * sizeof(ZcJob), cudaMemcpyHostToDevice, st));
     if (!fjobs.empty()) SP1_CUDA(cudaMemcpyAsync(d_fjobs, fjobs.data(), fjobs.size() * sizeof(ZcFixJob), cudaMemcpyHostToDevice, st));
-    SP1_TRY(mem.alloc((void**)&d_partial, (size_t)max_blocks * 36 * 4));
-    if ((size_t)max_jobs * 36 > SP1_MAIL_WORDS) return sp1b200_set_error("zerocheck: %u chips exceed the mailbox payload", max_jobs);
+    SP1_TRY(mem.alloc((void**)&d_partial, (size_t)max_blocks * ZC_GRID_WORDS * 4));
+    if ((size_t)max_jobs * ZC_GRID_WORDS > SP1_MAIL_WORDS) return sp1b200_set_error("zerocheck: %u chips exceed the mailbox payload", max_jobs);
     d_sums = sp1b200_mail_dev(ctx);
     SP1_CUDA(cudaMemsetAsync(d_final, 0, (wsum ? wsum : 1) * 16, st));
     void* d_ws = nullptr;
     if (ws_bytes) SP1_TRY(mem.alloc(&d_ws, ws_bytes));
-    auto launch_sum = [&](const Launch& Lc, bool ext, uint32_t* part) -> sp1b200_err {
+    auto launch_sum = [&](const Launch& Lc, int rd, uint32_t* part) -> sp1b200_err {
+        const bool ext = rd > 0;
         auto go = [&](auto kern, size_t smem) -> sp1b200_err {
             if (smem > 32 * 1024) SP1_CUDA(cudaFuncSetAttribute(kern, cudaFuncAttributeMaxDynamicSharedMemorySize, (int)smem));
             SP1_LAUNCH(ctx, kern, Lc.blocks, ZC_BLOCK, smem, d_jobs + Lc.job0, (int)Lc.n_jobs, m->d_chips, d_pv, d_gw, d_E[ecur], part, d_ws,
                        Lc.regs);
             return nullptr;
         };
+        if (grid && rd == 0) {
+            if (Lc.tier == 4) return go(zc_grid_kernel<RF_GLOBAL>, 0);
+            if (Lc.tier == 3) return go(zc_grid_kernel<RF_LOCAL>, 0);
+            return go(zc_grid_kernel<RF_SMEM>, (size_t)Lc.regs * ZC_GRID_NODES * ZC_BLOCK * 4);
+        }
         if (Lc.tier == 4) return ext ? go(zc_sum_kernel<Ext, RF_GLOBAL, false>, 0) : go(zc_sum_kernel<uint32_t, RF_GLOBAL, true>, 0);
         if (Lc.tier == 3) return ext ? go(zc_sum_kernel<Ext, RF_LOCAL, false>, 0) : go(zc_sum_kernel<uint32_t, RF_LOCAL, true>, 0);
         const size_t regs = Lc.regs;
@@ -674,29 +792,46 @@
     words.push_back(mlr);
     std::vector<E4> point;
     std::vector<E4> ys((size_t)nchips * 4);
-    std::vector<uint32_t> hs((size_t)max_jobs * 36);
+    std::vector<uint32_t> hs((size_t)max_jobs * ZC_GRID_WORDS);
     std::vector<E4> chip_sums(nchips * 9);
+    std::vector<E4> grid_sums(grid ? nchips * 16 : 0), grid_pad(grid ? nchips : 0);
     const E4 two = E4::from_base(hf::to_monty(2)), four = E4::from_base(hf::to_monty(4)), three = E4::from_base(hf::to_monty(3));
     for (uint32_t rd = 0; rd < mlr; rd++) {
         const RoundPlan& R = plan[rd];
+        const bool grid_pass = grid && rd == 0;
+        const uint32_t nw = grid_pass ? ZC_GRID_WORDS : 36;
         {
             uint32_t blk = 0, seq = 0; size_t jb = 0;
             for (const Launch& Lc : R.sums) {
-                SP1_TRY(launch_sum(Lc, rd > 0, d_partial + (size_t)blk * 36));
+                SP1_TRY(launch_sum(Lc, (int)rd, d_partial + (size_t)blk * nw));
                 const Mail mail = sp1b200_mail_next(ctx); seq = mail.seq;
-                SP1_LAUNCH(ctx, zc_reduce_kernel, Lc.n_jobs, 128, 0, d_jobs + Lc.job0, d_partial + (size_t)blk * 36, d_sums + jb * 36, mail);
+                if (grid_pass) SP1_LAUNCH(ctx, zc_reduce_kernel<ZC_GRID_WORDS>, Lc.n_jobs, 128, 0, d_jobs + Lc.job0, d_partial + (size_t)blk * nw, d_sums + jb * nw, mail);
+                else SP1_LAUNCH(ctx, zc_reduce_kernel<36>, Lc.n_jobs, 128, 0, d_jobs + Lc.job0, d_partial + (size_t)blk * nw, d_sums + jb * nw, mail);
                 blk += Lc.blocks; jb += Lc.n_jobs;
             }
             if (jb) {
                 HostSpan sp(acc_wait);
                 SP1_TRY(sp1b200_mail_wait(ctx, seq));
-                memcpy(hs.data(), sp1b200_mail_host(ctx), jb * 36 * 4);
+                memcpy(hs.data(), sp1b200_mail_host(ctx), jb * nw * 4);
             }
         }
         HostSpan sp_math(acc_math);
         std::fill(chip_sums.begin(), chip_sums.end(), E4());
-        for (size_t j = 0; j < R.chip_of_job.size(); j++)
-            for (int w9 = 0; w9 < 9; w9++) chip_sums[(size_t)R.chip_of_job[j] * 9 + w9] = chip_sums[(size_t)R.chip_of_job[j] * 9 + w9] + E4::load(&hs[j * 36 + 4 * w9]);
+        if (grid_pass) {
+            for (size_t j = 0; j < R.chip_of_job.size(); j++)
+                for (int w = 0; w < 16; w++) grid_sums[(size_t)R.chip_of_job[j] * 16 + w] = grid_sums[(size_t)R.chip_of_job[j] * 16 + w] + E4::load(&hs[j * nw + 4 * w]);
+            for (size_t k = 0; k < nchips; k++) {
+                if (!S[k].h) continue;
+                grid_pad[k] = S[k].pra * eq_at(gp, mlr - 2, (S[k].h + 3) / 4 - 1);
+                zc_grid_round0(&grid_sums[k * 16], gp[mlr - 2], S[k].h, grid_pad[k], &chip_sums[k * 9]);
+            }
+        } else if (grid && rd == 1) {
+            for (size_t k = 0; k < nchips; k++)
+                if (S[k].h) zc_grid_round1(&grid_sums[k * 16], point[0], h_heights[k], grid_pad[k], &chip_sums[k * 9]);
+        } else {
+            for (size_t j = 0; j < R.chip_of_job.size(); j++)
+                for (int w9 = 0; w9 < 9; w9++) chip_sums[(size_t)R.chip_of_job[j] * 9 + w9] = chip_sums[(size_t)R.chip_of_job[j] * 9 + w9] + E4::load(&hs[j * nw + 4 * w9]);
+        }
         const E4 last = gp[mlr - 1 - rd];
         const E4 bnode = (E4::one() - last) * hf::inv(E4::one() - (last + last));
         const E4 nodes[5] = {E4(), E4::one(), two, four, bnode};
@@ -715,14 +850,7 @@
                 E4 y2 = q[3] + (B + B) - A;
                 E4 y4 = q[6] + B * four - A * three;
                 const uint64_t th = (s.h + 1) / 2 - 1;
-                const uint64_t esize = (uint64_t)1 << (s.zeta.size() - 1);
-                E4 eth;
-                if (th < esize) {
-                    const size_t kk = s.zeta.size() - 1;
-                    eth = E4::one();
-                    for (size_t t = 0; t < kk; t++) eth = eth * (((th >> (kk - 1 - t)) & 1) ? s.zeta[t] : E4::one() - s.zeta[t]);
-                }
-                const E4 msb = s.eq_adj * eth;
+                const E4 msb = s.eq_adj * eq_at(s.zeta, s.zeta.size() - 1, th);
                 const E4 v0 = s.vg.fix_last(E4()).at(th), v2 = s.vg.fix_last(two).at(th), v4 = s.vg.fix_last(four).at(th);
                 y0 = y0 * (f0 * s.eq_adj) - s.pra * v0 * msb * f0;
                 y2 = y2 * (f2 * s.eq_adj) - s.pra * v2 * msb * f2;
@@ -740,10 +868,9 @@
         point.insert(point.begin(), a);
         const Ext da = to_ext(a);
         if (R.fix_jobs) {
-            if (rd == 0) {
-                SP1_LAUNCH(ctx, zc_fix_kernel<uint32_t>, R.fix_blocks, 256, 0, d_fjobs + R.fix0, (int)R.fix_jobs, da);
-                if (!bjobs.empty()) SP1_LAUNCH(ctx, zc_batch0_kernel, batch_blocks, 256, 0, d_bjobs, (int)bjobs.size(), d_gw, da);
-            } else SP1_LAUNCH(ctx, zc_fix_kernel<Ext>, R.fix_blocks, 256, 0, d_fjobs + R.fix0, (int)R.fix_jobs, da);
+            if (grid && rd == 1) SP1_LAUNCH(ctx, zc_fold2_kernel, R.fix_blocks, 256, 0, d_fjobs + R.fix0, (int)R.fix_jobs, to_ext(point[1]), da);
+            else if (rd == 0) SP1_LAUNCH(ctx, zc_fix_kernel<uint32_t>, R.fix_blocks, 256, 0, d_fjobs + R.fix0, (int)R.fix_jobs, da);
+            else SP1_LAUNCH(ctx, zc_fix_kernel<Ext>, R.fix_blocks, 256, 0, d_fjobs + R.fix0, (int)R.fix_jobs, da);
         }
         E4 La[4];
         for (int i = 0; i < 4; i++) La[i] = hf::eval_poly<5>(basis[i], a);
@@ -757,7 +884,7 @@
             s.zeta.pop_back();
             s.h = (s.h + 1) / 2;
         }
-        if (rd + 1 < mlr) {
+        if (rd + 1 < mlr && !grid_pass) {
             const uint64_t n_out = (uint64_t)1 << (mlr - 2 - rd);
             SP1_TRY(launch_halve_eq(ctx, d_E[ecur], n_out, d_E[ecur ^ 1]));
             ecur ^= 1;
```

New measurement: 64.76 million, median of 6. About the same (-0.0%).
